# YichengDWu/tinyedm

Hardware: AMD Instinct MI355X
Metric: train imgs/sec CIFAR-10 32x32 bf16 (higher is better)
Workload: dtype bf16; 1 GPU; CIFAR-10 32x32 unconditional EDM2 U-Net (conf/cifar10.yaml, 35.6M params) full training step: diffuse+embed+denoiser fwd/bwd+loss+grad all-reduce+Adam+EMA; per_gpu_batch=128, global_batch=128, parallelism=dp1, conditional=False, step_launch=hipGraph replay, collective=none

## Files before the change

### tinyedm_amd/csrc/elementwise.hip

```cpp
#include "common.h"
#include <stdarg.h>
#include <stdio.h>

static thread_local char g_err[512] = "";
extern "C" void edm_set_error(const char* fmt, ...) {
  va_list ap;
  va_start(ap, fmt);
  vsnprintf(g_err, sizeof(g_err), fmt, ap);
  va_end(ap);
}
extern "C" const char* edm_last_error() { return g_err; }
extern "C" int edm_version() { return 1; }

static inline int cdiv(long a, long b) { return (int)((a + b - 1) / b); }
static inline int grid_for(long work, int block, int cap = 256 * 16) {
  long g = (work + block - 1) / block;
  if (g > cap) g = cap;
  if (g < 1) g = 1;
  return (int)g;
}

template <int LPP, bool POOL = false>
__global__ __launch_bounds__(256) void k_pnorm_silu_fwd(const bf16* __restrict__ x, bf16* __restrict__ xn,
                                                          bf16* __restrict__ a, float* __restrict__ dsave, int P,
                                                          int C, int Hp = 0, int Wp = 0) {
  constexpr int GPW = 64 / LPP;
  const int lane = threadIdx.x & 63, wave = threadIdx.x >> 6;
  const int lig = lane % LPP, grp = lane / LPP;
  const int CL = C >> 3;
  const float rsC = rsqrtf((float)C);
  const long stride = (long)gridDim.x * 4 * GPW;
  for (long p0 = ((long)blockIdx.x * 4 + wave) * GPW; p0 < P; p0 += stride) {
    const long p = p0 + grp;
    const bool pv = p < P;
    float v[2][8];
    float ss = 0.f;
#pragma unroll
    for (int it = 0; it < 2; ++it) {
      const int c8 = lig + it * LPP;
      if (pv && c8 < CL) {
        if constexpr (POOL) {
          const int w = (int)(p % Wp);
          const long t = p / Wp;
          const int h = (int)(t % Hp);
          const long b = t / Hp;
          const bf16* src = x + ((b * 2 * Hp + 2 * h) * 2 * Wp + 2 * w) * C + c8 * 8;
          const long row = (long)2 * Wp * C;
          float a1[8], a2[8], a3[8];
          load8(src, v[it]);
          load8(src + C, a1);
          load8(src + row, a2);
          load8(src + row + C, a3);
#pragma unroll
          for (int i = 0; i < 8; ++i) v[it][i] = (float)(bf16)(0.25f * (v[it][i] + a1[i] + a2[i] + a3[i]));
        } else {
          load8(x + p * C + c8 * 8, v[it]);
        }
#pragma unroll
        for (int i = 0; i < 8; ++i) ss += v[it][i] * v[it][i];
      }
    }
    ss = group_sum<LPP>(ss);
    const float d = NORM_EPS + sqrtf(ss) * rsC;
    const float inv = 1.0f / d;
#pragma unroll
    for (int it = 0; it < 2; ++it) {
      const int c8 = lig + it * LPP;
      if (pv && c8 < CL) {
        float o[8], s[8];
#pragma unroll
        for (int i = 0; i < 8; ++i) {
          o[i] = (float)(bf16)(v[it][i] * inv);
          s[i] = mp_silu_b(o[i]);
        }
        store8(xn + p * C + c8 * 8, o);
        store8(a + p * C + c8 * 8, s);
      }
    }
    if (pv && lig == 0) dsave[p] = d;
  }
}

template <int LPP, bool UP = false>
__global__ __launch_bounds__(256) void k_pnorm_silu_bwd(const bf16* __restrict__ xn, const float* __restrict__ dsave,
                                                          const bf16* __restrict__ gxn, float gs,
                                                          const bf16* __restrict__ ga, const bf16* __restrict__ gadd,
                                                          bf16* __restrict__ gx, int P, int C, int Hp = 0, int Wp = 0) {
  constexpr int GPW = 64 / LPP;
  const int lane = threadIdx.x & 63, wave = threadIdx.x >> 6;
  const int lig = lane % LPP, grp = lane / LPP;
  const int CL = C >> 3;
  const long stride = (long)gridDim.x * 4 * GPW;
  for (long p0 = ((long)blockIdx.x * 4 + wave) * GPW; p0 < P; p0 += stride) {
    const long p = p0 + grp;
    const bool pv = p < P;
    float y[2][8], g[2][8];
    float dot = 0.f;
#pragma unroll
    for (int it = 0; it < 2; ++it) {
      const int c8 = lig + it * LPP;
      if (pv && c8 < CL) {
        load8(xn + p * C + c8 * 8, y[it]);
        float t[8];
        if (gxn) {
          load8(gxn + p * C + c8 * 8, t);
#pragma unroll
          for (int i = 0; i < 8; ++i) g[it][i] = gs * t[i];
        } else {
#pragma unroll
          for (int i = 0; i < 8; ++i) g[it][i] = 0.f;
        }
        if (ga) {
          load8(ga + p * C + c8 * 8, t);
#pragma unroll
          for (int i = 0; i < 8; ++i) g[it][i] += mp_silu_grad_b(y[it][i]) * t[i];
        }
#pragma unroll
        for (int i = 0; i < 8; ++i) dot += g[it][i] * y[it][i];
      }
    }
    dot = group_sum<LPP>(dot);
    float d = pv ? dsave[p] : 1.f;
    float s = d - NORM_EPS;
    float coef = s > 0.f ? dot * d / ((float)C * s) : 0.f;
    float inv = 1.0f / d;
#pragma unroll
    for (int it = 0; it < 2; ++it) {
      const int c8 = lig + it * LPP;
      if (pv && c8 < CL) {
        float o[8];
#pragma unroll
        for (int i = 0; i < 8; ++i) o[i] = (g[it][i] - y[it][i] * coef) * inv;
        if constexpr (UP) {
          const int w = (int)(p % Wp);
          const long t2 = p / Wp;
          const int h = (int)(t2 % Hp);
          const long b = t2 / Hp;
          const long e0 = ((b * 2 * Hp + 2 * h) * 2 * Wp + 2 * w) * C + c8 * 8;
          const long row = (long)2 * Wp * C;
#pragma unroll
          for (int i = 0; i < 8; ++i) o[i] = 0.25f * (float)(bf16)o[i];
#pragma unroll
          for (int q = 0; q < 4; ++q) {
            const long e = e0 + (q >> 1) * row + (q & 1) * C;
            float r[8];
#pragma unroll
            for (int i = 0; i < 8; ++i) r[i] = o[i];
            if (gadd) {
              float t[8];
              load8(gadd + e, t);
#pragma unroll
              for (int i = 0; i < 8; ++i) r[i] += t[i];
            }
            store8(gx + e, r);
          }
          continue;
        }
        if (gadd) {
          float t[8];
          load8(gadd + p * C + c8 * 8, t);
#pragma unroll
          for (int i = 0; i < 8; ++i) o[i] += t[i];
        }
        store8(gx + p * C + c8 * 8, o);
      }
    }
  }
}

static int pick_lpp(int C) {
  int cl = C / 8;
  return cl <= 16 ? 16 : (cl <= 32 ? 32 : 64);
}

extern "C" int edm_pixelnorm_silu_fwd(const void* x, void* xn, void* a, float* dsave, long P, int C,
                                      hipStream_t st) {
  EDM_REQUIRE(P > 0 && P < (1L << 31) && C > 0 && C % 8 == 0 && C <= 1024, "pixelnorm_silu_fwd: bad P=%ld C=%d", P, C);
  int lpp = pick_lpp(C);
  int gpw = 64 / lpp;
  int grid = grid_for(P, 4 * gpw);
#define L(N) hipLaunchKernelGGL(k_pnorm_silu_fwd<N>, dim3(grid), dim3(256), 0, st, (const bf16*)x, (bf16*)xn, (bf16*)a, dsave, (int)P, C)
  if (lpp == 16) L(16); else if (lpp == 32) L(32); else L(64);
#undef L
  EDM_CHECK_LAUNCH("pixelnorm_silu_fwd");
  return EDM_OK;
}

extern "C" int edm_pool_pixelnorm_silu_fwd(const void* x, void* xn, void* a, float* dsave, int B, int Hp, int Wp, int C,
                                           hipStream_t st) {
  EDM_REQUIRE(x && xn && a && dsave && B > 0 && Hp > 0 && Wp > 0 && C > 0 && C % 8 == 0 && C <= 1024 &&
                  (long)B * Hp * Wp < (1L << 31), "pool_pixelnorm_silu_fwd: bad args");
  const long P = (long)B * Hp * Wp;
  int lpp = pick_lpp(C);
  int gpw = 64 / lpp;
  int grid = grid_for(P, 4 * gpw);
#define L(N) hipLaunchKernelGGL((k_pnorm_silu_fwd<N, true>), dim3(grid), dim3(256), 0, st, (const bf16*)x, (bf16*)xn, (bf16*)a, dsave, (int)P, C, Hp, Wp)
  if (lpp == 16) L(16); else if (lpp == 32) L(32); else L(64);
#undef L
  EDM_CHECK_LAUNCH("pool_pixelnorm_silu_fwd");
  return EDM_OK;
}
extern "C" int edm_pool_pixelnorm_silu_bwd(const void* xn, const float* dsave, const void* gxn, float gxn_scale,
                                           const void* ga, const void* gadd, void* gx, int B, int Hp, int Wp, int C,
                                           hipStream_t st) {
  EDM_REQUIRE(xn && dsave && gx && B > 0 && Hp > 0 && Wp > 0 && C > 0 && C % 8 == 0 && C <= 1024 &&
                  (long)B * Hp * Wp < (1L << 31), "pool_pixelnorm_silu_bwd: bad args");
  const long P = (long)B * Hp * Wp;
  int lpp = pick_lpp(C);
  int gpw = 64 / lpp;
  int grid = grid_for(P, 4 * gpw);
#define L(N) hipLaunchKernelGGL((k_pnorm_silu_bwd<N, true>), dim3(grid), dim3(256), 0, st, (const bf16*)xn, dsave, (const bf16*)gxn, gxn_scale, (const bf16*)ga, (const bf16*)gadd, (bf16*)gx, (int)P, C, Hp, Wp)
  if (lpp == 16) L(16); else if (lpp == 32) L(32); else L(64);
#undef L
  EDM_CHECK_LAUNCH("pool_pixelnorm_silu_bwd");
  return EDM_OK;
}

extern "C" int edm_pixelnorm_silu_bwd(const void* xn, const float* dsave, const void* gxn, float gxn_scale,
                                      const void* ga, const void* gadd, void* gx, long P, int C, hipStream_t st) {
  EDM_REQUIRE(P > 0 && P < (1L << 31) && C > 0 && C % 8 == 0 && C <= 1024, "pixelnorm_silu_bwd: bad P=%ld C=%d", P, C);
  int lpp = pick_lpp(C);
  int gpw = 64 / lpp;
  int grid = grid_for(P, 4 * gpw);
#define L(N) hipLaunchKernelGGL(k_pnorm_silu_bwd<N>, dim3(grid), dim3(256), 0, st, (const bf16*)xn, dsave, (const bf16*)gxn, gxn_scale, (const bf16*)ga, (const bf16*)gadd, (bf16*)gx, (int)P, C)
  if (lpp == 16) L(16); else if (lpp == 32) L(32); else L(64);
#undef L
  EDM_CHECK_LAUNCH("pixelnorm_silu_bwd");
  return EDM_OK;
}

__global__ void k_silu_fwd(const bf16* __restrict__ x, bf16* __restrict__ a, long n8) {
  for (long i = (long)blockIdx.x * blockDim.x + threadIdx.x; i < n8; i += (long)gridDim.x * blockDim.x) {
    float v[8];
    load8(x + i * 8, v);
#pragma unroll
    for (int j = 0; j < 8; ++j) v[j] = mp_silu_b(v[j]);
    store8(a + i * 8, v);
  }
}
__global__ void k_silu_bwd(const bf16* __restrict__ x, const bf16* __restrict__ ga, const bf16* __restrict__ ge,
                           float s, bf16* __restrict__ gx, long n8) {
  for (long i = (long)blockIdx.x * blockDim.x + threadIdx.x; i < n8; i += (long)gridDim.x * blockDim.x) {
    float v[8], g[8], e[8];
    load8(x + i * 8, v);
    load8(ga + i * 8, g);
    if (ge) load8(ge + i * 8, e);
#pragma unroll
    for (int j = 0; j < 8; ++j) g[j] = mp_silu_grad_b(v[j]) * g[j] + (ge ? s * e[j] : 0.f);
    store8(gx + i * 8, g);
  }
}
extern "C" int edm_silu_fwd(const void* x, void* a, long n, hipStream_t st) {
  EDM_REQUIRE(n > 0 && n % 8 == 0, "silu_fwd: n=%ld must be a positive multiple of 8", n);
  hipLaunchKernelGGL(k_silu_fwd, dim3(grid_for(n / 8, 256)), dim3(256), 0, st, (const bf16*)x, (bf16*)a, n / 8);
  EDM_CHECK_LAUNCH("silu_fwd");
  return EDM_OK;
}
extern "C" int edm_silu_bwd(const void* x, const void* ga, const void* gextra, float extra_scale, void* gx, long n,
                            hipStream_t st) {
  EDM_REQUIRE(n > 0 && n % 8 == 0, "silu_bwd: n=%ld must be a positive multiple of 8", n);
  hipLaunchKernelGGL(k_silu_bwd, dim3(grid_for(n / 8, 256)), dim3(256), 0, st, (const bf16*)x, (const bf16*)ga,
                     (const bf16*)gextra, extra_scale, (bf16*)gx, n / 8);
  EDM_CHECK_LAUNCH("silu_bwd");
  return EDM_OK;
}

__global__ void k_axpby(const bf16* __restrict__ a, float alpha, const bf16* __restrict__ b, float beta,
                        bf16* __restrict__ o, long n8) {
  for (long i = (long)blockIdx.x * blockDim.x + threadIdx.x; i < n8; i += (long)gridDim.x * blockDim.x) {
    float u[8], v[8];
    load8(a + i * 8, u);
    if (b) load8(b + i * 8, v);
#pragma unroll
    for (int j = 0; j < 8; ++j) u[j] = alpha * u[j] + (b ? beta * v[j] : 0.f);
    store8(o + i * 8, u);
  }
}
extern "C" int edm_axpby(const void* a, float alpha, const void* b, float beta, void* out, long n, hipStream_t st) {
  EDM_REQUIRE(n > 0 && n % 8 == 0, "axpby: n=%ld must be a positive multiple of 8", n);
  hipLaunchKernelGGL(k_axpby, dim3(grid_for(n / 8, 256)), dim3(256), 0, st, (const bf16*)a, alpha, (const bf16*)b,
                     beta, (bf16*)out, n / 8);
  EDM_CHECK_LAUNCH("axpby");
  return EDM_OK;
}


__global__ void k_mod_silu_drop_fwd(const bf16* __restrict__ r, const float* __restrict__ lin,
                                    const float* __restrict__ gain, bf16* __restrict__ a, int HW, int C, long n8,
                                    long lin_stride, float pdrop, uint32_t seed_lo, uint32_t seed_hi, uint32_t sub, uint32_t step,
                                    const StepParams* __restrict__ dyn) {
  if (dyn) { step = dyn->step; seed_lo = dyn->seed_lo; seed_hi = dyn->seed_hi; }
  const int CL = C >> 3;
  const float g = *gain;
  for (long i = (long)blockIdx.x * blockDim.x + threadIdx.x; i < n8; i += (long)gridDim.x * blockDim.x) {
    const int c8 = (int)(i % CL);
    const long pix = i / CL;
    const int b = (int)(pix / HW);
    float v[8];
    load8(r + i * 8, v);
    const float* lp = lin + (long)b * lin_stride + c8 * 8;
    const Keep8 keep = dropout_keep8(i, pdrop, sub, step, seed_lo, seed_hi);
    const float keep_scale = keep.scale;
#pragma unroll
    for (int j = 0; j < 8; ++j) {
      float m = lp[j] * g + 1.0f;
      float o = mp_silu_b(v[j] * m);
      if (pdrop > 0.f) o = keep[j] ? o * keep_scale : 0.f;
      v[j] = o;
    }
    store8(a + i * 8, v);
  }
}

__global__ void k_mod_silu_drop_bwd(const bf16* __restrict__ r, const float* __restrict__ lin,
                                    const float* __restrict__ gain, const bf16* __restrict__ ga,
                                    bf16* __restrict__ gr, float* __restrict__ gm, long gm_stride, int HW, int C, int PIXW,
                                    long lin_stride, float pdrop, uint32_t seed_lo, uint32_t seed_hi, uint32_t sub, uint32_t step,
                                    const StepParams* __restrict__ dyn) {
  extern __shared__ __attribute__((aligned(16))) float red[];
  if (dyn) { step = dyn->step; seed_lo = dyn->seed_lo; seed_hi = dyn->seed_hi; }
  const int CL = C >> 3;
  const int PS = blockDim.x / CL;
  const int c8 = threadIdx.x % CL, ps = threadIdx.x / CL;
  const int b = blockIdx.x;
  const int p_begin = blockIdx.y * PIXW;
  const int p_end = min(HW, p_begin + PIXW);
  const float g = *gain;
  float m[8], acc[8];
#pragma unroll
  for (int j = 0; j < 8; ++j) {
    m[j] = lin[(long)b * lin_stride + c8 * 8 + j] * g + 1.0f;
    acc[j] = 0.f;
  }
  for (int p = p_begin + ps; p < p_end; p += PS) {
    const long i = ((long)b * HW + p) * CL + c8;
    float v[8], gg[8];
    load8(r + i * 8, v);
    load8(ga + i * 8, gg);
    const Keep8 keep = dropout_keep8(i, pdrop, sub, step, seed_lo, seed_hi);
    const float keep_scale = keep.scale;
#pragma unroll
    for (int j = 0; j < 8; ++j) {
      const float u = (pdrop > 0.f && !keep[j]) ? 0.f : v[j];
      float gu = gg[j] * mp_silu_grad_b(u * m[j]);
      if (pdrop > 0.f) gu = keep[j] ? gu * keep_scale : 0.f;
      acc[j] += gu * u;
      gg[j] = gu * m[j];
    }
    store8(gr + i * 8, gg);
  }
#pragma unroll
  for (int j = 0; j < 8; ++j) red[ps * C + c8 * 8 + j] = acc[j];
  __syncthreads();
  for (int c = threadIdx.x; c < C; c += blockDim.x) {
    float s = 0.f;
    for (int q = 0; q < PS; ++q) s += red[q * C + c];
    atomicAdd(gm + (long)b * gm_stride + c, s);
  }
}
__global__ void k_mod_finish(const float* __restrict__ gm, const float* __restrict__ lin,
                             const float* __restrict__ gain, float* __restrict__ glin, float* __restrict__ ggain,
                             long n, int C, long lin_stride, long glin_stride) {
  const float g = *gain;
  float part = 0.f;
  for (long i = (long)blockIdx.x * blockDim.x + threadIdx.x; i < n; i += (long)gridDim.x * blockDim.x) {
    const long b = i / C;
    const int c = (int)(i - b * C);
    float v = gm[i];
    glin[b * glin_stride + c] = v * g;
    part += v * lin[b * lin_stride + c];
  }
  part = wave_sum(part);
  if ((threadIdx.x & 63) == 0) atomicAdd(ggain, part);
}

static int block_for_chunks(int CL) { return (256 / CL) * CL; }

extern "C" int edm_mod_silu_drop_fwd(const void* r, const float* lin, long lin_stride, const float* gain, void* a, int B,
                                     int HW, int C, float pdrop, unsigned long long seed, unsigned sub, unsigned step,
                                     const void* dyn, hipStream_t st) {
  EDM_REQUIRE(B > 0 && HW > 0 && C % 8 == 0 && C > 0 && pdrop >= 0.f && pdrop < 1.f && lin_stride >= C,
              "mod_silu_drop_fwd: bad args");
  long n8 = (long)B * HW * C / 8;
  hipLaunchKernelGGL(k_mod_silu_drop_fwd, dim3(grid_for(n8, 256)), dim3(256), 0, st, (const bf16*)r, lin, gain,
                     (bf16*)a, HW, C, n8, lin_stride, pdrop, (uint32_t)seed, (uint32_t)(seed >> 32), sub, step,
                     (const StepParams*)dyn);
  EDM_CHECK_LAUNCH("mod_silu_drop_fwd");
  return EDM_OK;
}

extern "C" int edm_mod_silu_drop_bwd(const void* r, const float* lin, long lin_stride, const float* gain,
                                     const void* ga, void* gr, float* gm, float* glin, long glin_stride, float* ggain,
                                     int B, int HW, int C, float pdrop, unsigned long long seed, unsigned sub,
                                     unsigned step, const void* dyn, hipStream_t st) {
  EDM_REQUIRE(B > 0 && HW > 0 && C % 8 == 0 && C > 0 && C <= 1024 && lin_stride >= C && glin_stride >= C,
              "mod_silu_drop_bwd: bad args");
  int CL = C / 8, block = block_for_chunks(CL), PS = block / CL;
  int PIXW = HW >= 256 ? 128 : HW;
  hipLaunchKernelGGL(k_mod_silu_drop_bwd, dim3(B, cdiv(HW, PIXW)), dim3(block), PS * C * sizeof(float), st,
                     (const bf16*)r, lin, gain, (const bf16*)ga, (bf16*)gr, gm, (long)C, HW, C, PIXW, lin_stride, pdrop,
                     (uint32_t)seed, (uint32_t)(seed >> 32), sub, step, (const StepParams*)dyn);
  EDM_CHECK_LAUNCH("mod_silu_drop_bwd");
  hipLaunchKernelGGL(k_mod_finish, dim3(grid_for((long)B * C, 256, 64)), dim3(256), 0, st, gm, lin, gain, glin,
                     ggain, (long)B * C, C, lin_stride, glin_stride);
  EDM_CHECK_LAUNCH("mod_finish");
  return EDM_OK;
}

extern "C" int edm_mod_silu_drop_bwd_raw(const void* r, const float* lin, long lin_stride, const float* gain,
                                         const void* ga, void* gr, float* gm, long gm_stride, int B, int HW, int C,
                                         float pdrop, unsigned long long seed, unsigned sub, unsigned step,
                                         const void* dyn, hipStream_t st) {
  EDM_REQUIRE(r && lin && gain && ga && gr && gm, "mod_silu_drop_bwd_raw: null pointer");
  EDM_REQUIRE(B > 0 && HW > 0 && C % 8 == 0 && C > 0 && C <= 1024 && lin_stride >= C && gm_stride >= C,
              "mod_silu_drop_bwd_raw: bad args");
  int CL = C / 8, block = block_for_chunks(CL), PS = block / CL;
  int PIXW = HW >= 256 ? 128 : HW;
  hipLaunchKernelGGL(k_mod_silu_drop_bwd, dim3(B, cdiv(HW, PIXW)), dim3(block), PS * C * sizeof(float), st,
                     (const bf16*)r, lin, gain, (const bf16*)ga, (bf16*)gr, gm, gm_stride, HW, C, PIXW, lin_stride, pdrop,
                     (uint32_t)seed, (uint32_t)(seed >> 32), sub, step, (const StepParams*)dyn);
  EDM_CHECK_LAUNCH("mod_silu_drop_bwd_raw");
  return EDM_OK;
}

extern "C" int edm_mod_finish(const float* gm, const float* lin, long lin_stride, const float* gain, float* glin,
                              long glin_stride, float* ggain, int B, int C, hipStream_t st) {
  EDM_REQUIRE(gm && lin && gain && glin && ggain && B > 0 && C > 0 && lin_stride >= C && glin_stride >= C,
              "mod_finish: bad args");
  hipLaunchKernelGGL(k_mod_finish, dim3(grid_for((long)B * C, 256, 64)), dim3(256), 0, st, gm, lin, gain, glin, ggain,
                     (long)B * C, C, lin_stride, glin_stride);
  EDM_CHECK_LAUNCH("mod_finish");
  return EDM_OK;
}

struct ModFinItem {
  const float* gain;
  float* ggain;
  int col0, C;
};
__global__ void k_mod_finish_multi(const float* __restrict__ gm, const float* __restrict__ lin, float* __restrict__ glin,
                                   long stride, const ModFinItem* __restrict__ items, int B) {
  const ModFinItem it = items[blockIdx.x];
  const float g = *it.gain;
  const long n = (long)B * it.C;
  float part = 0.f;
  for (long i = (long)blockIdx.y * blockDim.x + threadIdx.x; i < n; i += (long)gridDim.y * blockDim.x) {
    const long b = i / it.C;
    const long e = b * stride + it.col0 + (i - b * it.C);
    const float v = gm[e];
    glin[e] += v * g;
    part += v * lin[e];
  }
  __shared__ float red[4];
  part = wave_sum(part);
  if ((threadIdx.x & 63) == 0) red[threadIdx.x >> 6] = part;
  __syncthreads();
  if (threadIdx.x == 0) atomicAdd(it.ggain, red[0] + red[1] + red[2] + red[3]);
}
extern "C" int edm_mod_finish_multi(const float* gm_all, const float* lin_all, float* glin_all, long stride,
                                    const void* items_dev, int n_items, int B, hipStream_t st) {
  EDM_REQUIRE(gm_all && lin_all && glin_all && items_dev && n_items > 0 && n_items <= 4096 && B > 0 && stride > 0,
              "mod_finish_multi: bad args");
  hipLaunchKernelGGL(k_mod_finish_multi, dim3(n_items, 8), dim3(256), 0, st, gm_all, lin_all, glin_all, stride,
                     (const ModFinItem*)items_dev, B);
  EDM_CHECK_LAUNCH("mod_finish_multi");
  return EDM_OK;
}

__global__ void k_dropout_mask(uint8_t* __restrict__ mask, long n8, float pdrop, uint32_t seed_lo, uint32_t seed_hi,
                               uint32_t sub, uint32_t step) {
  for (long i = (long)blockIdx.x * blockDim.x + threadIdx.x; i < n8; i += (long)gridDim.x * blockDim.x) {
    const Keep8 keep = dropout_keep8(i, pdrop, sub, step, seed_lo, seed_hi);
#pragma unroll
    for (int j = 0; j < 8; ++j) mask[i * 8 + j] = keep[j] ? 1 : 0;
  }
}
extern "C" int edm_dropout_mask(unsigned char* mask, long n, float pdrop, unsigned long long seed, unsigned sub,
                                unsigned step, hipStream_t st) {
  EDM_REQUIRE(n > 0 && n % 8 == 0, "dropout_mask: n must be a multiple of 8");
  hipLaunchKernelGGL(k_dropout_mask, dim3(grid_for(n / 8, 256)), dim3(256), 0, st, mask, n / 8, pdrop,
                     (uint32_t)seed, (uint32_t)(seed >> 32), sub, step);
  EDM_CHECK_LAUNCH("dropout_mask");
  return EDM_OK;
}

__global__ void k_pool2(const bf16* __restrict__ x, bf16* __restrict__ y, int H, int W, int CL, long n8, float s) {
  for (long i = (long)blockIdx.x * blockDim.x + threadIdx.x; i < n8; i += (long)gridDim.x * blockDim.x) {
    int c8 = (int)(i % CL);
    long pix = i / CL;
    int w = (int)(pix % W);
    long t = pix / W;
    int h = (int)(t % H);
    long b = t / H;
    const long row = (long)2 * W * CL;
    const bf16* src = x + (((b * 2 * H + 2 * h) * 2 * W + 2 * w) * CL + c8) * 8;
    float a0[8], a1[8], a2[8], a3[8];
    load8(src, a0);
    load8(src + CL * 8, a1);
    load8(src + row * 8, a2);
    load8(src + row * 8 + CL * 8, a3);
#pragma unroll
    for (int j = 0; j < 8; ++j) a0[j] = s * (a0[j] + a1[j] + a2[j] + a3[j]);
    store8(y + i * 8, a0);
  }
}
__global__ void k_up2(const bf16* __restrict__ x, const bf16* __restrict__ add, bf16* __restrict__ y, int H, int W, int CL,
                      long n8, float s) {
  for (long i = (long)blockIdx.x * blockDim.x + threadIdx.x; i < n8; i += (long)gridDim.x * blockDim.x) {
    int c8 = (int)(i % CL);
    long pix = i / CL;
    int w = (int)(pix % W);
    long t = pix / W;
    int h = (int)(t % H);
    long b = t / H;
    const bf16* src = x + (((b * (H / 2) + h / 2) * (W / 2) + w / 2) * CL + c8) * 8;
    float a0[8];
    load8(src, a0);
    if (s != 1.0f) {
#pragma unroll
      for (int j = 0; j < 8; ++j) a0[j] *= s;
    }
    if (add) {
      float t[8];
      load8(add + i * 8, t);
#pragma unroll
      for (int j = 0; j < 8; ++j) a0[j] += t[j];
    }
    store8(y + i * 8, a0);
  }
}
__global__ void k_up2_silu(const bf16* __restrict__ x, bf16* __restrict__ y, bf16* __restrict__ a, int H, int W, int CL,
                           long n8) {
  for (long i = (long)blockIdx.x * blockDim.x + threadIdx.x; i < n8; i += (long)gridDim.x * blockDim.x) {
    int c8 = (int)(i % CL);
    long pix = i / CL;
    int w = (int)(pix % W);
    long t = pix / W;
    int h = (int)(t % H);
    long b = t / H;
    const u32x4 raw = *reinterpret_cast<const u32x4*>(x + (((b * (H / 2) + h / 2) * (W / 2) + w / 2) * CL + c8) * 8);
    *reinterpret_cast<u32x4*>(y + i * 8) = raw;
    const bf16x8 v = __builtin_bit_cast(bf16x8, raw);
    float f[8];
#pragma unroll
    for (int j = 0; j < 8; ++j) f[j] = mp_silu_b((float)v[j]);
    store8(a + i * 8, f);
  }
}
extern "C" int edm_up2_silu(const void* x, void* y, void* a, int B, int Hout, int Wout, int C, hipStream_t st) {
  EDM_REQUIRE(x && y && a && B > 0 && Hout > 0 && Wout > 0 && Hout % 2 == 0 && Wout % 2 == 0 && C % 8 == 0, "up2_silu: bad args");
  long n8 = (long)B * Hout * Wout * C / 8;
  hipLaunchKernelGGL(k_up2_silu, dim3(grid_for(n8, 256)), dim3(256), 0, st, (const bf16*)x, (bf16*)y, (bf16*)a, Hout, Wout,
                     C / 8, n8);
  EDM_CHECK_LAUNCH("up2_silu");
  return EDM_OK;
}
extern "C" int edm_pool2(const void* x, void* y, int B, int Hout, int Wout, int C, float scale, hipStream_t st) {
  EDM_REQUIRE(B > 0 && Hout > 0 && Wout > 0 && C % 8 == 0, "pool2: bad args");
  long n8 = (long)B * Hout * Wout * C / 8;
  hipLaunchKernelGGL(k_pool2, dim3(grid_for(n8, 256)), dim3(256), 0, st, (const bf16*)x, (bf16*)y, Hout, Wout, C / 8,
                     n8, scale);
  EDM_CHECK_LAUNCH("pool2");
  return EDM_OK;
}
extern "C" int edm_up2(const void* x, const void* add, void* y, int B, int Hout, int Wout, int C, float scale,
                       hipStream_t st) {
  EDM_REQUIRE(B > 0 && Hout > 0 && Wout > 0 && Hout % 2 == 0 && Wout % 2 == 0 && C % 8 == 0, "up2: bad args");
  long n8 = (long)B * Hout * Wout * C / 8;
  hipLaunchKernelGGL(k_up2, dim3(grid_for(n8, 256)), dim3(256), 0, st, (const bf16*)x, (const bf16*)add, (bf16*)y, Hout,
                     Wout, C / 8, n8, scale);
  EDM_CHECK_LAUNCH("up2");
  return EDM_OK;
}

__global__ __launch_bounds__(256) void k_reduce_hw_det(const bf16* __restrict__ x, long xs, const bf16* __restrict__ y,
                                                         long ys, float* __restrict__ out, int HW, int C, float scale) {
  __shared__ float red[32][65];
  const int b = blockIdx.x, c0 = blockIdx.y * 64;
  const int cl = threadIdx.x & 7, pl = threadIdx.x >> 3;
  const int c = c0 + cl * 8;
  const bool cok = c < C;
  float acc[8] = {0, 0, 0, 0, 0, 0, 0, 0};
  const long base = (long)b * HW;
  constexpr int UN = 16;
  for (int p0 = pl; p0 < HW; p0 += 32 * UN) {
    u32x4 v[UN], u[UN];
#pragma unroll
    for (int k = 0; k < UN; ++k) {
      const int p = p0 + 32 * k;
      const bool ok = cok && p < HW;
      v[k] = ok ? *reinterpret_cast<const u32x4*>(x + (base + p) * xs + c) : u32x4{0u, 0u, 0u, 0u};
      if (y) u[k] = ok ? *reinterpret_cast<const u32x4*>(y + (base + p) * ys + c) : u32x4{0u, 0u, 0u, 0u};
    }
#pragma unroll
    for (int k = 0; k < UN; ++k) {
      const bf16x8 a = __builtin_bit_cast(bf16x8, v[k]);
      if (y) {
        const bf16x8 b = __builtin_bit_cast(bf16x8, u[k]);
#pragma unroll
        for (int j = 0; j < 8; ++j) acc[j] += (float)a[j] * (float)b[j];
      } else {
#pragma unroll
        for (int j = 0; j < 8; ++j) acc[j] += (float)a[j];
      }
    }
  }
#pragma unroll
  for (int j = 0; j < 8; ++j) red[pl][cl * 8 + j] = acc[j];
  __syncthreads();
  if (threadIdx.x < 64 && c0 + (int)threadIdx.x < C) {
    float s = 0.f;
#pragma unroll
    for (int q = 0; q < 32; ++q) s += red[q][threadIdx.x];
    out[(long)b * C + c0 + threadIdx.x] = s * scale;
  }
}
extern "C" int edm_reduce_hw(const void* x, long x_stride, const void* y, long y_stride, float* out, int B, int HW,
                             int C, float scale, hipStream_t st) {
  EDM_REQUIRE(B > 0 && HW > 0 && C % 8 == 0 && C > 0 && C <= 4096 && x_stride % 8 == 0 && y_stride % 8 == 0,
              "reduce_hw: bad args");
  hipLaunchKernelGGL(k_reduce_hw_det, dim3(B, cdiv(C, 64)), dim3(256), 0, st, (const bf16*)x, x_stride, (const bf16*)y,
                     y_stride, out, HW, C, scale);
  EDM_CHECK_LAUNCH("reduce_hw");
  return EDM_OK;
}

__device__ __forceinline__ float strided_dot(const float* __restrict__ w, long stride, const float* v, int n) {
  float s = 0.f;
  int r = 0;
  for (; r + 16 <= n; r += 16) {
    float t[16];
#pragma unroll
    for (int k = 0; k < 16; ++k) t[k] = w[(long)(r + k) * stride];
#pragma unroll
    for (int k = 0; k < 16; ++k) s += t[k] * v[r + k];
  }
  for (; r < n; ++r) s += w[(long)r * stride] * v[r];
  return s;
}

__global__ void k_scalelong_fwd(const float* __restrict__ mean, const float* __restrict__ W1, const float* __restrict__ W2,
                                float* __restrict__ gate, float* __restrict__ z1save, int C, int R) {
  extern __shared__ __attribute__((aligned(16))) float sm[];
  float* m = sm;
  float* h = sm + C + 1;
  const int b = blockIdx.x;
  for (int c = threadIdx.x; c < C; c += blockDim.x) m[c] = mean[(long)b * C + c];
  if (threadIdx.x == 0) m[C] = 1.0f;
  __syncthreads();
  const int lane = threadIdx.x & 63, wave = threadIdx.x >> 6, nw = blockDim.x >> 6;
  for (int r = wave; r < R; r += nw) {
    float s = 0.f;
    for (int c = lane; c <= C; c += 64) s += W1[(long)r * (C + 1) + c] * m[c];
    s = wave_sum(s);
    if (lane == 0) {
      z1save[(long)b * R + r] = s;
      h[r] = mp_silu_f(s);
    }
  }
  __syncthreads();
  for (int c = threadIdx.x; c < C; c += blockDim.x) gate[(long)b * C + c] = sigmoidf_(strided_dot(W2 + (long)c * R, 1, h, R));
}
__global__ void k_scalelong_bwd(const float* __restrict__ mean, const float* __restrict__ W1, const float* __restrict__ W2,
                                const float* __restrict__ gate, const float* __restrict__ z1save,
                                const float* __restrict__ ggate, float* __restrict__ gmean, float* __restrict__ gW1,
                                float* __restrict__ gW2, int C, int R) {
  extern __shared__ __attribute__((aligned(16))) float sm[];
  float* m = sm;
  float* h = m + C + 1;
  float* gz2 = h + R;
  float* gz1 = gz2 + C;
  const int b = blockIdx.x;
  for (int c = threadIdx.x; c < C; c += blockDim.x) {
    m[c] = mean[(long)b * C + c];
    float g = gate[(long)b * C + c];
    gz2[c] = ggate[(long)b * C + c] * g * (1.0f - g);
  }
  if (threadIdx.x == 0) m[C] = 1.0f;
  for (int r = threadIdx.x; r < R; r += blockDim.x) h[r] = mp_silu_f(z1save[(long)b * R + r]);
  __syncthreads();
  for (int i = threadIdx.x; i < C * R; i += blockDim.x) atomicAdd(gW2 + i, gz2[i / R] * h[i % R]);
  const int lane = threadIdx.x & 63, wave = threadIdx.x >> 6, nw = blockDim.x >> 6;
  for (int r = wave; r < R; r += nw) {
    float s = 0.f;
    for (int c = lane; c < C; c += 64) s += W2[(long)c * R + r] * gz2[c];
    s = wave_sum(s);
    if (lane == 0) gz1[r] = s * mp_silu_grad_f(z1save[(long)b * R + r]);
  }
  __syncthreads();
  for (int i = threadIdx.x; i < R * (C + 1); i += blockDim.x) atomicAdd(gW1 + i, gz1[i / (C + 1)] * m[i % (C + 1)]);
  for (int c = threadIdx.x; c < C; c += blockDim.x) {
    float s = 0.f;
    for (int r = 0; r < R; ++r) s += W1[(long)r * (C + 1) + c] * gz1[r];
    gmean[(long)b * C + c] = s;
  }
}
extern "C" int edm_scalelong_fwd(const float* mean, const float* W1h, const float* W2h, float* gate, float* z1save,
                                 int B, int C, int R, hipStream_t st) {
  EDM_REQUIRE(B > 0 && C > 0 && R > 0 && C <= 4096, "scalelong_fwd: bad args");
  hipLaunchKernelGGL(k_scalelong_fwd, dim3(B), dim3(256), (C + 1 + R) * sizeof(float), st, mean, W1h, W2h, gate,
                     z1save, C, R);
  EDM_CHECK_LAUNCH("scalelong_fwd");
  return EDM_OK;
}
extern "C" int edm_scalelong_bwd(const float* mean, const float* W1h, const float* W2h, const float* gate,
                                 const float* z1save, const float* ggate, float* gmean, float* gW1h, float* gW2h,
                                 int B, int C, int R, hipStream_t st) {
  EDM_REQUIRE(B > 0 && C > 0 && R > 0 && C <= 4096, "scalelong_bwd: bad args");
  hipLaunchKernelGGL(k_scalelong_bwd, dim3(B), dim3(256), (2 * C + 1 + 2 * R) * sizeof(float), st, mean, W1h, W2h,
                     gate, z1save, ggate, gmean, gW1h, gW2h, C, R);
  EDM_CHECK_LAUNCH("scalelong_bwd");
  return EDM_OK;
}

template <bool MUL>
__device__ __forceinline__ void sample_reduce(const bf16* __restrict__ x, long xs, const bf16* __restrict__ y, long ys,
                                              int HW, int C, float* red, float* out_lds, float scale) {
  const int lpr = C >> 3;
  const int rpp = blockDim.x / lpr;
  const int cl = threadIdx.x % lpr, rg = threadIdx.x / lpr;
  float acc[8] = {0, 0, 0, 0, 0, 0, 0, 0};
  if (rg < rpp) {
    constexpr int UN = 8;
    for (int p0 = rg; p0 < HW; p0 += rpp * UN) {
      u32x4 v[UN], u[UN];
#pragma unroll
      for (int k = 0; k < UN; ++k) {
        const int p = p0 + rpp * k;
        const bool ok = p < HW;
        v[k] = ok ? *reinterpret_cast<const u32x4*>(x + (long)p * xs + cl * 8) : u32x4{0u, 0u, 0u, 0u};
        if (MUL) u[k] = ok ? *reinterpret_cast<const u32x4*>(y + (long)p * ys + cl * 8) : u32x4{0u, 0u, 0u, 0u};
      }
#pragma unroll
      for (int k = 0; k < UN; ++k) {
        const bf16x8 a = __builtin_bit_cast(bf16x8, v[k]);
        if (MUL) {
          const bf16x8 b = __builtin_bit_cast(bf16x8, u[k]);
#pragma unroll
          for (int j = 0; j < 8; ++j) acc[j] += (float)a[j] * (float)b[j];
        } else {
#pragma unroll
          for (int j = 0; j < 8; ++j) acc[j] += (float)a[j];
        }
      }
    }
#pragma unroll
    for (int j = 0; j < 8; ++j) red[rg * C + cl * 8 + j] = acc[j];
  }
  __syncthreads();
  for (int c = threadIdx.x; c < C; c += blockDim.x) {
    float s = 0.f;
    for (int q = 0; q < rpp; ++q) s += red[q * C + c];
    out_lds[c] = s * scale;
  }
  __syncthreads();
}

template <bool KEEP = false>
__device__ __forceinline__ void skip_gate_fwd_body(const bf16* __restrict__ skip, const float* __restrict__ W1,
                                                   const float* __restrict__ W2, float* __restrict__ mean,
                                                   float* __restrict__ gate, float* __restrict__ z1save, int HW,
                                                   int C, int R, int b) {
  extern __shared__ __attribute__((aligned(16))) float sm[];
  const int rpp = blockDim.x / (C >> 3);
  float* red = sm;
  float* m = sm + rpp * C;
  float* h = m + C + 1;
  sample_reduce<false>(skip + (long)b * HW * C, C, nullptr, 0, HW, C, red, m, 1.0f / (float)HW);
  for (int c = threadIdx.x; c < C; c += blockDim.x) mean[(long)b * C + c] = m[c];
  if (threadIdx.x == 0) m[C] = 1.0f;
  __syncthreads();
  const int lane = threadIdx.x & 63, wave = threadIdx.x >> 6, nw = blockDim.x >> 6;
  for (int r = wave < nw ? wave : R; r < R; r += nw) {
    float s = 0.f;
    for (int c = lane; c <= C; c += 64) s += W1[(long)r * (C + 1) + c] * m[c];
    s = wave_sum(s);
    if (lane == 0) {
      z1save[(long)b * R + r] = s;
      h[r] = mp_silu_f(s);
    }
  }
  __syncthreads();
  for (int c = threadIdx.x; c < C; c += blockDim.x) {
    const float gv = sigmoidf_(strided_dot(W2 + (long)c * R, 1, h, R));
    gate[(long)b * C + c] = gv;
    if (KEEP) red[c] = gv;
  }
}
__global__ __launch_bounds__(1024) void k_skip_gate_fwd(const bf16* __restrict__ skip, const float* __restrict__ W1,
                                                          const float* __restrict__ W2, float* __restrict__ mean,
                                                          float* __restrict__ gate, float* __restrict__ z1save, int HW,
                                                          int C, int R) {
  skip_gate_fwd_body(skip, W1, W2, mean, gate, z1save, HW, C, R, blockIdx.x);
}
constexpr int MAXSGF = 32;
struct SgfItem {
  const bf16* skip;
  const float* W1;
  const float* W2;
  float* mean;
  float* gate;
  float* z1;
  bf16* cat;
  bf16* sil;
  int Ci, pad;
  int B, HW, R, blk0;
};
struct SgfGroup {
  SgfItem it[MAXSGF];
  int n, C, pad[2];
};
__global__ __launch_bounds__(1024) void k_skip_gate_fwd_multi(const SgfGroup* __restrict__ g) {
  int k = 0;
  const int n = g->n;
  while (k + 1 < n && (int)blockIdx.x >= g->it[k + 1].blk0) ++k;
  const SgfItem it = g->it[k];
  const int C = g->C, b = (int)blockIdx.x - it.blk0;
  skip_gate_fwd_body<true>(it.skip, it.W1, it.W2, it.mean, it.gate, it.z1, it.HW, C, it.R, b);
  if (it.cat == nullptr) return;
  __syncthreads();
  extern __shared__ __attribute__((aligned(16))) float sm[];
  const int CLs = C >> 3;
  const long ld = it.Ci + C;
  const bf16* __restrict__ sk = it.skip + (long)b * it.HW * C;
  bf16* __restrict__ cat = it.cat + (long)b * it.HW * ld + it.Ci;
  bf16* __restrict__ sil = it.sil ? it.sil + (long)b * it.HW * ld + it.Ci : nullptr;
  const int n8 = it.HW * CLs;
  for (int i = threadIdx.x; i < n8; i += blockDim.x) {
    const int cs = (i % CLs) * 8;
    const int pix = i / CLs;
    float v[8];
    load8(sk + (long)pix * C + cs, v);
#pragma unroll
    for (int j = 0; j < 8; ++j) v[j] = (float)(bf16)(v[j] * sm[cs + j]);
    store8(cat + (long)pix * ld + cs, v);
    if (sil) {
#pragma unroll
      for (int j = 0; j < 8; ++j) v[j] = mp_silu_b(v[j]);
      store8(sil + (long)pix * ld + cs, v);
    }
  }
}
__device__ __forceinline__ void skip_gate_bwd_body(const bf16* __restrict__ gcat, long gs, const bf16* __restrict__ skip,
                                                   const float* __restrict__ W1, const float* __restrict__ W2,
                                                   const float* __restrict__ gate, const float* __restrict__ z1save,
                                                   float* __restrict__ gmean, float* __restrict__ ws, int HW, int C,
                                                   int R, int b) {
  extern __shared__ __attribute__((aligned(16))) float sm[];
  const int rpp = blockDim.x / (C >> 3);
  float* red = sm;
  float* gz2 = sm + rpp * C;
  float* gz1 = gz2 + C;
  float* wsb = ws + (long)b * (C + 2 * R);
  sample_reduce<true>(gcat + (long)b * HW * gs, gs, skip + (long)b * HW * C, C, HW, C, red, gz2, 1.0f);
  for (int c = threadIdx.x; c < C; c += blockDim.x) {
    const float g = gate[(long)b * C + c];
    gz2[c] *= g * (1.0f - g);
    wsb[c] = gz2[c];
  }
  for (int r = threadIdx.x; r < R; r += blockDim.x) wsb[C + R + r] = mp_silu_f(z1save[(long)b * R + r]);
  __syncthreads();
  const int lane = threadIdx.x & 63, wave = threadIdx.x >> 6, nw = blockDim.x >> 6;
  for (int r = wave < nw ? wave : R; r < R; r += nw) {
    float s = 0.f;
    for (int c = lane; c < C; c += 64) s += W2[(long)c * R + r] * gz2[c];
    s = wave_sum(s);
    if (lane == 0) {
      gz1[r] = s * mp_silu_grad_f(z1save[(long)b * R + r]);
      wsb[C + r] = gz1[r];
    }
  }
  __syncthreads();
  for (int c = threadIdx.x; c < C; c += blockDim.x) gmean[(long)b * C + c] = strided_dot(W1 + c, C + 1, gz1, R);
}
__global__ __launch_bounds__(1024) void k_skip_gate_bwd(const bf16* __restrict__ gcat, long gs, const bf16* __restrict__ skip,
                                                          const float* __restrict__ W1, const float* __restrict__ W2,
                                                          const float* __restrict__ gate, const float* __restrict__ z1save,
                                                          float* __restrict__ gmean, float* __restrict__ ws, int HW, int C,
                                                          int R) {
  skip_gate_bwd_body(gcat, gs, skip, W1, W2, gate, z1save, gmean, ws, HW, C, R, blockIdx.x);
}
struct SgbItem {
  const bf16* gcat;
  long gs;
  const bf16* skip;
  const float* W1;
  const float* W2;
  const float* gate;
  const float* z1;
  float* gmean;
  float* ws;
  bf16* gskip;
  int B, HW, R, blk0;
};
struct SgbGroup {
  SgbItem it[MAXSGF];
  int n, C, pad[2];
};
__global__ __launch_bounds__(1024) void k_skip_gate_bwd_multi(const SgbGroup* __restrict__ g) {
  int k = 0;
  const int n = g->n;
  while (k + 1 < n && (int)blockIdx.x >= g->it[k + 1].blk0) ++k;
  const SgbItem it = g->it[k];
  const int C = g->C, b = (int)blockIdx.x - it.blk0;
  skip_gate_bwd_body(it.gcat, it.gs, it.skip, it.W1, it.W2, it.gate, it.z1, it.gmean, it.ws, it.HW, C, it.R, b);
  if (it.gskip == nullptr) return;
  __syncthreads();
  const int CLs = C >> 3;
  const float inv_hw = 1.0f / (float)it.HW;
  const bf16* __restrict__ gc = it.gcat + (long)b * it.HW * it.gs;
  bf16* __restrict__ out = it.gskip + (long)b * it.HW * C;
  const float* gp0 = it.gate + (long)b * C;
  const float* mp0 = it.gmean + (long)b * C;
  const int n8 = it.HW * CLs;
  for (int i = threadIdx.x; i < n8; i += blockDim.x) {
    const int cs = (i % CLs) * 8;
    const int pix = i / CLs;
    float v[8];
    load8(gc + (long)pix * it.gs + cs, v);
    const float* gp = gp0 + cs;
    const float* mp = mp0 + cs;
#pragma unroll
    for (int j = 0; j < 8; ++j) v[j] = v[j] * gp[j] + mp[j] * inv_hw;
    store8(out + (long)pix * C + cs, v);
  }
}
__device__ __forceinline__ void skip_gate_wgrad_body(const float* __restrict__ ws, const float* __restrict__ mean,
                                                     float* __restrict__ gW1, float* __restrict__ gW2, int B, int C, int R,
                                                     int CT, int BC, int blk) {
  extern __shared__ __attribute__((aligned(16))) float sm[];
  float* A = sm;
  float* Bm = sm + 4 * BC;
  const int W = C + 2 * R;
  const bool second = blk >= CT;
  const int c0 = (second ? blk - CT : blk) * 4;
  const int ncol = second ? C + 1 : C;
  const int boff = second ? C : C + R;
  constexpr int MAXO = 16;
  float acc[MAXO];
#pragma unroll
  for (int k = 0; k < MAXO; ++k) acc[k] = 0.f;
  for (int b0 = 0; b0 < B; b0 += BC) {
    const int nb = min(BC, B - b0);
    if (b0) __syncthreads();
    for (int i = threadIdx.x; i < 4 * nb; i += blockDim.x) {
      const int b = b0 + (i >> 2), c = c0 + (i & 3);
      float v = 0.f;
      if (c < ncol) v = second ? (c < C ? mean[(long)b * C + c] : 1.0f) : ws[(long)b * W + c];
      A[i] = v;
    }
    for (int i = threadIdx.x; i < nb * R; i += blockDim.x) Bm[i] = ws[(long)(b0 + i / R) * W + boff + i % R];
    __syncthreads();
#pragma unroll
    for (int k = 0; k < MAXO; ++k) {
      const int o = threadIdx.x + k * 256;
      if (o < 4 * R) {
        const int cc = o / R, r = o % R;
        float s = acc[k];
        for (int b = 0; b < nb; ++b) s += A[b * 4 + cc] * Bm[b * R + r];
        acc[k] = s;
      }
    }
  }
#pragma unroll
  for (int k = 0; k < MAXO; ++k) {
    const int o = threadIdx.x + k * 256;
    if (o >= 4 * R) continue;
    const int cc = o / R, r = o % R;
    if (c0 + cc >= ncol) continue;
    if (second) gW1[(long)r * (C + 1) + c0 + cc] = acc[k];
    else gW2[(long)(c0 + cc) * R + r] = acc[k];
  }
}
__global__ __launch_bounds__(256) void k_skip_gate_wgrad(const float* __restrict__ ws, const float* __restrict__ mean,
                                                           float* __restrict__ gW1, float* __restrict__ gW2, int B, int C,
                                                           int R, int CT, int BC) {
  skip_gate_wgrad_body(ws, mean, gW1, gW2, B, C, R, CT, BC, blockIdx.x);
}
constexpr int MAXSG = 32;
struct SgItem {
  const float* ws;
  const float* mean;
  float* gW1;
  float* gW2;
  int B, C, R, blk0;
};
struct SgGroup {
  SgItem it[MAXSG];
  int n, pad[3];
};
__global__ __launch_bounds__(256) void k_skip_gate_wgrad_multi(const SgGroup* __restrict__ g) {
  int k = 0;
  const int n = g->n;
  while (k + 1 < n && (int)blockIdx.x >= g->it[k + 1].blk0) ++k;
  const SgItem it = g->it[k];
  const int CT = (it.C + 3) / 4;
  const int BC = it.B < 16384 / (it.R + 4) ? it.B : 16384 / (it.R + 4);
  skip_gate_wgrad_body(it.ws, it.mean, it.gW1, it.gW2, it.B, it.C, it.R, CT, BC, (int)blockIdx.x - it.blk0);
}
static inline int skip_gate_threads(int C) {
  const int lpr = C / 8;
  int t = 1024 / lpr * lpr;
  return t < 64 ? 0 : t;
}
extern "C" int edm_skip_gate_fwd(const void* skip, const float* W1h, const float* W2h, float* mean, float* gate,
                                 float* z1save, int B, int HW, int C, int R, hipStream_t st) {
  EDM_REQUIRE(skip && W1h && W2h && mean && gate && z1save, "skip_gate_fwd: null pointer");
  EDM_REQUIRE(B > 0 && HW > 0 && C > 0 && C % 8 == 0 && C <= 4096 && R > 0 && R <= 1024, "skip_gate_fwd: bad args");
  const int threads = skip_gate_threads(C);
  EDM_REQUIRE(threads > 0, "skip_gate_fwd: C too large");
  const size_t lds = ((size_t)(threads / (C / 8)) * C + C + 1 + R) * sizeof(float);
  hipLaunchKernelGGL(k_skip_gate_fwd, dim3(B), dim3(threads), lds, st, (const bf16*)skip, W1h, W2h, mean, gate, z1save,
                     HW, C, R);
  EDM_CHECK_LAUNCH("skip_gate_fwd");
  return EDM_OK;
}
struct edm_skip_gate_fwd_item_ {
  const void* skip;
  const float* W1h;
  const float* W2h;
  float* mean;
  float* gate;
  float* z1save;
  void* cat;
  void* silu_out;
  int B, HW, C, R, Ci, pad;
};
extern "C" long edm_skip_gate_fwd_multi_table_bytes(void) { return (long)sizeof(SgfGroup); }
extern "C" int edm_skip_gate_fwd_multi(const void* items_, int n, void* table_host, void* table_dev, int defer_upload,
                                       hipStream_t st) {
  const edm_skip_gate_fwd_item_* items = (const edm_skip_gate_fwd_item_*)items_;
  EDM_REQUIRE(items && n > 0 && n <= MAXSGF, "skip_gate_fwd_multi: need 1..%d gates, got %d", MAXSGF, n);
  SgfGroup g;
  g.n = n;
  g.C = items[0].C;
  g.pad[0] = g.pad[1] = 0;
  const int C = g.C;
  EDM_REQUIRE(C > 0 && C % 8 == 0 && C <= 4096, "skip_gate_fwd_multi: bad channel count %d", C);
  const int threads = skip_gate_threads(C);
  EDM_REQUIRE(threads > 0, "skip_gate_fwd_multi: C too large");
  long blk = 0;
  int rmax = 0;
  for (int k = 0; k < n; ++k) {
    const edm_skip_gate_fwd_item_& a = items[k];
    EDM_REQUIRE(a.skip && a.W1h && a.W2h && a.mean && a.gate && a.z1save, "skip_gate_fwd_multi: null pointer (gate %d)", k);
    EDM_REQUIRE(a.C == C, "skip_gate_fwd_multi: the gates of one launch share a channel count (%d vs %d)", a.C, C);
    EDM_REQUIRE(a.B > 0 && a.HW > 0 && a.R > 0 && a.R <= 1024, "skip_gate_fwd_multi: bad item %d", k);
    EDM_REQUIRE(a.cat ? (a.Ci > 0 && a.Ci % 8 == 0) : (a.silu_out == nullptr),
                "skip_gate_fwd_multi: cat needs Ci %% 8 == 0 (gate %d); silu_out needs cat", k);
    g.it[k] = SgfItem{(const bf16*)a.skip, a.W1h, a.W2h, a.mean, a.gate, a.z1save, (bf16*)a.cat, (bf16*)a.silu_out, a.Ci, 0,
                      a.B, a.HW, a.R, (int)blk};
    blk += a.B;
    EDM_REQUIRE(blk < (1L << 30), "skip_gate_fwd_multi: grid too large");
    if (a.R > rmax) rmax = a.R;
  }
  for (int k = n; k < MAXSGF; ++k)
    g.it[k] = SgfItem{nullptr, nullptr, nullptr, nullptr, nullptr, nullptr, nullptr, nullptr, 0, 0, 0, 0, 0, (int)blk};
  const size_t lds = ((size_t)(threads / (C / 8)) * C + C + 1 + rmax) * sizeof(float);
  EDM_UPLOAD_TABLE(table_dev, table_host, &g, sizeof(SgfGroup), st, "skip_gate_fwd_multi", defer_upload);
  hipLaunchKernelGGL(k_skip_gate_fwd_multi, dim3((unsigned)blk), dim3(threads), lds, st, (const SgfGroup*)table_dev);
  EDM_CHECK_LAUNCH("skip_gate_fwd_multi");
  return EDM_OK;
}
extern "C" int edm_skip_gate_bwd(const void* gcat, long gcat_stride, int c_off, const void* skip, const float* mean,
                                 const float* W1h, const float* W2h, const float* gate, const float* z1save, float* gmean,
                                 float* gW1h, float* gW2h, float* ws, int B, int HW, int C, int R, hipStream_t st) {
  EDM_REQUIRE(gcat && skip && mean && W1h && W2h && gate && z1save && gmean && ws && (!gW1h == !gW2h), "skip_gate_bwd: null pointer");
  EDM_REQUIRE(B > 0 && HW > 0 && C > 0 && C % 8 == 0 && C <= 4096 && R > 0 && R <= 1024 && c_off >= 0 && c_off % 8 == 0 &&
                  gcat_stride >= c_off + C && gcat_stride % 8 == 0, "skip_gate_bwd: bad args");
  const int threads = skip_gate_threads(C);
  EDM_REQUIRE(threads > 0, "skip_gate_bwd: C too large");
  const size_t lds = ((size_t)(threads / (C / 8)) * C + C + R) * sizeof(float);
  hipLaunchKernelGGL(k_skip_gate_bwd, dim3(B), dim3(threads), lds, st, (const bf16*)gcat + c_off, gcat_stride,
                     (const bf16*)skip, W1h, W2h, gate, z1save, gmean, ws, HW, C, R);
  if (gW1h) {
    const int CT = (C + 3) / 4, CT1 = (C + 4) / 4;
    const int BC = B < 16384 / (R + 4) ? B : 16384 / (R + 4);
    const size_t lds2 = ((size_t)4 * BC + (size_t)BC * R) * sizeof(float);
    hipLaunchKernelGGL(k_skip_gate_wgrad, dim3(CT + CT1), dim3(256), lds2, st, ws, mean, gW1h, gW2h, B, C, R, CT, BC);
  }
  EDM_CHECK_LAUNCH("skip_gate_bwd");
  return EDM_OK;
}

struct edm_skip_gate_bwd_item_ {
  const void* gcat;
  long gcat_stride;
  const void* skip;
  const float* W1h;
  const float* W2h;
  const float* gate;
  const float* z1save;
  float* gmean;
  float* ws;
  void* gskip;
  int c_off, B, HW, C, R, pad;
};
extern "C" int edm_skip_gate_bwd_multi(const void* items_, int n, void* table_host, void* table_dev, int defer_upload,
                                       hipStream_t st) {
  const edm_skip_gate_bwd_item_* items = (const edm_skip_gate_bwd_item_*)items_;
  EDM_REQUIRE(items && n > 0 && n <= MAXSGF, "skip_gate_bwd_multi: need 1..%d gates, got %d", MAXSGF, n);
  SgbGroup g;
  g.n = n;
  g.C = items[0].C;
  g.pad[0] = g.pad[1] = 0;
  const int C = g.C;
  EDM_REQUIRE(C > 0 && C % 8 == 0 && C <= 4096, "skip_gate_bwd_multi: bad channel count %d", C);
  const int threads = skip_gate_threads(C);
  EDM_REQUIRE(threads > 0, "skip_gate_bwd_multi: C too large");
  long blk = 0;
  int rmax = 0;
  for (int k = 0; k < n; ++k) {
    const edm_skip_gate_bwd_item_& a = items[k];
    EDM_REQUIRE(a.gcat && a.skip && a.W1h && a.W2h && a.gate && a.z1save && a.gmean && a.ws,
                "skip_gate_bwd_multi: null pointer (gate %d)", k);
    EDM_REQUIRE(a.C == C, "skip_gate_bwd_multi: the gates of one launch share a channel count (%d vs %d)", a.C, C);
    EDM_REQUIRE(a.B > 0 && a.HW > 0 && a.R > 0 && a.R <= 1024 && a.c_off >= 0 && a.c_off % 8 == 0 &&
                    a.gcat_stride >= a.c_off + C && a.gcat_stride % 8 == 0, "skip_gate_bwd_multi: bad item %d", k);
    g.it[k] = SgbItem{(const bf16*)a.gcat + a.c_off, a.gcat_stride, (const bf16*)a.skip, a.W1h, a.W2h, a.gate, a.z1save,
                      a.gmean, a.ws, (bf16*)a.gskip, a.B, a.HW, a.R, (int)blk};
    blk += a.B;
    EDM_REQUIRE(blk < (1L << 30), "skip_gate_bwd_multi: grid too large");
    if (a.R > rmax) rmax = a.R;
  }
  for (int k = n; k < MAXSGF; ++k)
    g.it[k] = SgbItem{nullptr, 0, nullptr, nullptr, nullptr, nullptr, nullptr, nullptr, nullptr, nullptr, 0, 0, 0, (int)blk};
  const size_t lds = ((size_t)(threads / (C / 8)) * C + C + rmax) * sizeof(float);
  EDM_UPLOAD_TABLE(table_dev, table_host, &g, sizeof(SgbGroup), st, "skip_gate_bwd_multi", defer_upload);
  hipLaunchKernelGGL(k_skip_gate_bwd_multi, dim3((unsigned)blk), dim3(threads), lds, st, (const SgbGroup*)table_dev);
  EDM_CHECK_LAUNCH("skip_gate_bwd_multi");
  return EDM_OK;
}
struct edm_skip_gate_wgrad_item_ {
  const float* ws;
  const float* mean;
  float* gW1h;
  float* gW2h;
  int B, C, R, pad;
};
extern "C" long edm_skip_gate_wgrad_multi_table_bytes(void) { return (long)sizeof(SgGroup); }
extern "C" int edm_skip_gate_wgrad_multi(const void* items_, int n, void* table_host, void* table_dev, int defer_upload,
                                         hipStream_t st) {
  const edm_skip_gate_wgrad_item_* items = (const edm_skip_gate_wgrad_item_*)items_;
  EDM_REQUIRE(items && n > 0 && n <= MAXSG, "skip_gate_wgrad_multi: need 1..%d gates, got %d", MAXSG, n);
  SgGroup g;
  g.n = n;
  int blk = 0;
  size_t lds = 0;
  for (int k = 0; k < n; ++k) {
    const edm_skip_gate_wgrad_item_& a = items[k];
    EDM_REQUIRE(a.ws && a.mean && a.gW1h && a.gW2h && a.B > 0 && a.C > 0 && a.C % 8 == 0 && a.C <= 4096 && a.R > 0 && a.R <= 1024,
                "skip_gate_wgrad_multi: bad item %d", k);
    g.it[k] = SgItem{a.ws, a.mean, a.gW1h, a.gW2h, a.B, a.C, a.R, blk};
    blk += (a.C + 3) / 4 + (a.C + 4) / 4;
    const int BC = a.B < 16384 / (a.R + 4) ? a.B : 16384 / (a.R + 4);
    const size_t need = ((size_t)4 * BC + (size_t)BC * a.R) * sizeof(float);
    if (need > lds) lds = need;
  }
  EDM_MAX_LDS(k_skip_gate_wgrad_multi, 128 * 1024);
  EDM_UPLOAD_TABLE(table_dev, table_host, &g, sizeof(SgGroup), st, "skip_gate_wgrad_multi", defer_upload);
  hipLaunchKernelGGL(k_skip_gate_wgrad_multi, dim3(blk), dim3(256), lds, st, (const SgGroup*)table_dev);
  EDM_CHECK_LAUNCH("skip_gate_wgrad_multi");
  return EDM_OK;
}

__global__ void k_concat_gate_fwd(const bf16* __restrict__ inp, const bf16* __restrict__ skip,
                                  const float* __restrict__ gate, bf16* __restrict__ cat, bf16* __restrict__ sil,
                                  int HW, int Ci, int Cs, long n8) {
  const int CLt = (Ci + Cs) >> 3, CLi = Ci >> 3;
  for (long i = (long)blockIdx.x * blockDim.x + threadIdx.x; i < n8; i += (long)gridDim.x * blockDim.x) {
    int c8 = (int)(i % CLt);
    long pix = i / CLt;
    float v[8];
    if (c8 < CLi) {
      load8(inp + pix * Ci + c8 * 8, v);
    } else {
      int cs = (c8 - CLi) * 8;
      int b = (int)(pix / HW);
      load8(skip + pix * Cs + cs, v);
      const float* gp = gate + (long)b * Cs + cs;
#pragma unroll
      for (int j = 0; j < 8; ++j) v[j] = (float)(bf16)(v[j] * gp[j]);
    }
    store8(cat + i * 8, v);
    if (sil) {
#pragma unroll
      for (int j = 0; j < 8; ++j) v[j] = mp_silu_b(v[j]);
      store8(sil + i * 8, v);
    }
  }
}
__global__ void k_concat_gate_bwd(const bf16* __restrict__ gcat, const float* __restrict__ gate,
                                  const float* __restrict__ gmean, bf16* __restrict__ ginp, bf16* __restrict__ gskip,
                                  int HW, int Ci, int Cs, long n8, float inv_hw) {
  const int CLt = (Ci + Cs) >> 3, CLi = Ci >> 3;
  for (long i = (long)blockIdx.x * blockDim.x + threadIdx.x; i < n8; i += (long)gridDim.x * blockDim.x) {
    int c8 = (int)(i % CLt);
    long pix = i / CLt;
    float v[8];
    load8(gcat + i * 8, v);
    if (c8 < CLi) {
      store8(ginp + pix * Ci + c8 * 8, v);
    } else {
      int cs = (c8 - CLi) * 8;
      int b = (int)(pix / HW);
      const float* gp = gate + (long)b * Cs + cs;
      const float* mp = gmean + (long)b * Cs + cs;
#pragma unroll
      for (int j = 0; j < 8; ++j) v[j] = v[j] * gp[j] + mp[j] * inv_hw;
      store8(gskip + pix * Cs + cs, v);
    }
  }
}
__global__ void k_skip_half_fwd(const bf16* __restrict__ skip, const float* __restrict__ gate, bf16* __restrict__ cat,
                                bf16* __restrict__ sil, int HW, int Ci, int Cs, long n8) {
  const int CLs = Cs >> 3;
  const long ld = Ci + Cs;
  for (long i = (long)blockIdx.x * blockDim.x + threadIdx.x; i < n8; i += (long)gridDim.x * blockDim.x) {
    const int cs = (int)(i % CLs) * 8;
    const long pix = i / CLs;
    const int b = (int)(pix / HW);
    float v[8];
    load8(skip + pix * Cs + cs, v);
    const float* gp = gate + (long)b * Cs + cs;
#pragma unroll
    for (int j = 0; j < 8; ++j) v[j] = (float)(bf16)(v[j] * gp[j]);
    store8(cat + pix * ld + Ci + cs, v);
    if (sil) {
#pragma unroll
      for (int j = 0; j < 8; ++j) v[j] = mp_silu_b(v[j]);
      store8(sil + pix * ld + Ci + cs, v);
    }
  }
}
__device__ __forceinline__ void skip_half_bwd_body(const bf16* __restrict__ gcs, const float* __restrict__ gate,
                                                   const float* __restrict__ gmean, bf16* __restrict__ gskip, int HW, int Cs,
                                                   long n8, float inv_hw, long first, long stride) {
  const int CLs = Cs >> 3;
  for (long i = first; i < n8; i += stride) {
    const int cs = (int)(i % CLs) * 8;
    const int b = (int)((i / CLs) / HW);
    float v[8];
    load8(gcs + i * 8, v);
    const float* gp = gate + (long)b * Cs + cs;
    const float* mp = gmean + (long)b * Cs + cs;
#pragma unroll
    for (int j = 0; j < 8; ++j) v[j] = v[j] * gp[j] + mp[j] * inv_hw;
    store8(gskip + i * 8, v);
  }
}
__global__ void k_skip_half_bwd(const bf16* __restrict__ gcs, const float* __restrict__ gate,
                                const float* __restrict__ gmean, bf16* __restrict__ gskip, int HW, int Cs, long n8,
                                float inv_hw) {
  skip_half_bwd_body(gcs, gate, gmean, gskip, HW, Cs, n8, inv_hw, (long)blockIdx.x * blockDim.x + threadIdx.x,
                     (long)gridDim.x * blockDim.x);
}
struct ShbItem {
  const bf16* gcs;
  const float* gate;
  const float* gmean;
  bf16* gskip;
  long n8;
  float inv_hw;
  int HW, Cs, blk0, nblk, pad;
};
struct ShbGroup {
  ShbItem it[MAXSGF];
  int n, pad[3];
};
__global__ void k_skip_half_bwd_multi(const ShbGroup* __restrict__ g) {
  int k = 0;
  const int n = g->n;
  while (k + 1 < n && (int)blockIdx.x >= g->it[k + 1].blk0) ++k;
  const ShbItem it = g->it[k];
  skip_half_bwd_body(it.gcs, it.gate, it.gmean, it.gskip, it.HW, it.Cs, it.n8, it.inv_hw,
                     (long)((int)blockIdx.x - it.blk0) * blockDim.x + threadIdx.x, (long)it.nblk * blockDim.x);
}
extern "C" int edm_skip_half_fwd(const void* skip, const float* gate, void* cat, void* silu_out, int B, int HW, int Ci,
                                 int Cs, hipStream_t st) {
  EDM_REQUIRE(skip && gate && cat, "skip_half_fwd: null pointer");
  EDM_REQUIRE(B > 0 && HW > 0 && Ci % 8 == 0 && Cs % 8 == 0 && Ci > 0 && Cs > 0, "skip_half_fwd: bad args");
  long n8 = (long)B * HW * Cs / 8;
  hipLaunchKernelGGL(k_skip_half_fwd, dim3(grid_for(n8, 256)), dim3(256), 0, st, (const bf16*)skip, gate, (bf16*)cat,
                     (bf16*)silu_out, HW, Ci, Cs, n8);
  EDM_CHECK_LAUNCH("skip_half_fwd");
  return EDM_OK;
}
extern "C" int edm_skip_half_bwd(const void* gcs, const float* gate, const float* gmean, void* gskip, int B, int HW, int Cs,
                                 hipStream_t st) {
  EDM_REQUIRE(gcs && gate && gmean && gskip, "skip_half_bwd: null pointer");
  EDM_REQUIRE(B > 0 && HW > 0 && Cs % 8 == 0 && Cs > 0, "skip_half_bwd: bad args");
  long n8 = (long)B * HW * Cs / 8;
  hipLaunchKernelGGL(k_skip_half_bwd, dim3(grid_for(n8, 256)), dim3(256), 0, st, (const bf16*)gcs, gate, gmean,
                     (bf16*)gskip, HW, Cs, n8, 1.0f / (float)HW);
  EDM_CHECK_LAUNCH("skip_half_bwd");
  return EDM_OK;
}
extern "C" long edm_skip_gate_bwd_multi_table_bytes(void) {
  return (long)(sizeof(SgbGroup) > sizeof(ShbGroup) ? sizeof(SgbGroup) : sizeof(ShbGroup));
}
struct edm_skip_half_bwd_item_ {
  const void* gcs;
  const float* gate;
  const float* gmean;
  void* gskip;
  int B, HW, Cs, pad;
};
extern "C" int edm_skip_half_bwd_multi(const void* items_, int n, void* table_host, void* table_dev, int defer_upload,
                                       hipStream_t st) {
  const edm_skip_half_bwd_item_* items = (const edm_skip_half_bwd_item_*)items_;
  EDM_REQUIRE(items && n > 0 && n <= MAXSGF, "skip_half_bwd_multi: need 1..%d tensors, got %d", MAXSGF, n);
  ShbGroup g;
  g.n = n;
  g.pad[0] = g.pad[1] = g.pad[2] = 0;
  long blk = 0;
  for (int k = 0; k < n; ++k) {
    const edm_skip_half_bwd_item_& a = items[k];
    EDM_REQUIRE(a.gcs && a.gate && a.gmean && a.gskip, "skip_half_bwd_multi: null pointer (tensor %d)", k);
    EDM_REQUIRE(a.B > 0 && a.HW > 0 && a.Cs % 8 == 0 && a.Cs > 0, "skip_half_bwd_multi: bad item %d", k);
    const long n8 = (long)a.B * a.HW * a.Cs / 8;
    const int nblk = grid_for(n8, 256);
    g.it[k] = ShbItem{(const bf16*)a.gcs, a.gate, a.gmean, (bf16*)a.gskip, n8, 1.0f / (float)a.HW, a.HW, a.Cs, (int)blk, nblk, 0};
    blk += nblk;
    EDM_REQUIRE(blk < (1L << 30), "skip_half_bwd_multi: grid too large");
  }
  for (int k = n; k < MAXSGF; ++k) g.it[k] = ShbItem{nullptr, nullptr, nullptr, nullptr, 0, 0.f, 1, 8, (int)blk, 0, 0};
  EDM_UPLOAD_TABLE(table_dev, table_host, &g, sizeof(ShbGroup), st, "skip_half_bwd_multi", defer_upload);
  hipLaunchKernelGGL(k_skip_half_bwd_multi, dim3((unsigned)blk), dim3(256), 0, st, (const ShbGroup*)table_dev);
  EDM_CHECK_LAUNCH("skip_half_bwd_multi");
  return EDM_OK;
}

extern "C" int edm_concat_gate_fwd(const void* inp, const void* skip, const float* gate, void* cat, void* silu_out,
                                   int B, int HW, int Ci, int Cs, hipStream_t st) {
  EDM_REQUIRE(B > 0 && HW > 0 && Ci % 8 == 0 && Cs % 8 == 0 && Ci > 0 && Cs > 0, "concat_gate_fwd: bad args");
  long n8 = (long)B * HW * (Ci + Cs) / 8;
  hipLaunchKernelGGL(k_concat_gate_fwd, dim3(grid_for(n8, 256)), dim3(256), 0, st, (const bf16*)inp,
                     (const bf16*)skip, gate, (bf16*)cat, (bf16*)silu_out, HW, Ci, Cs, n8);
  EDM_CHECK_LAUNCH("concat_gate_fwd");
  return EDM_OK;
}
extern "C" int edm_concat_gate_bwd(const void* gcat, const float* gate, const float* gmean, void* ginp, void* gskip,
                                   int B, int HW, int Ci, int Cs, hipStream_t st) {
  EDM_REQUIRE(B > 0 && HW > 0 && Ci % 8 == 0 && Cs % 8 == 0 && Ci > 0 && Cs > 0, "concat_gate_bwd: bad args");
  long n8 = (long)B * HW * (Ci + Cs) / 8;
  hipLaunchKernelGGL(k_concat_gate_bwd, dim3(grid_for(n8, 256)), dim3(256), 0, st, (const bf16*)gcat, gate, gmean,
                     (bf16*)ginp, (bf16*)gskip, HW, Ci, Cs, n8, 1.0f / (float)HW);
  EDM_CHECK_LAUNCH("concat_gate_bwd");
  return EDM_OK;
}

__global__ void k_precond_in(const float* __restrict__ noisy, const float* __restrict__ sigma, int sstride, float sd,
                             bf16* __restrict__ out, int Cimg, int HW, int CP, long npix) {
  for (long p = (long)blockIdx.x * blockDim.x + threadIdx.x; p < npix; p += (long)gridDim.x * blockDim.x) {
    long b = p / HW;
    int hw = (int)(p % HW);
    float s = sigma[b * sstride];
    float cin = rsqrtf(sd * sd + s * s);
    bf16* o = out + p * CP;
    for (int c0 = 0; c0 < CP; c0 += 8) {
      float v[8];
#pragma unroll
      for (int j = 0; j < 8; ++j) {
        int c = c0 + j;
        v[j] = c < Cimg ? cin * noisy[(b * Cimg + c) * HW + hw] : (c == Cimg ? 1.0f : 0.0f);
      }
      store8(o + c0, v);
    }
  }
}
extern "C" int edm_precond_in(const float* noisy, const float* sigma, int sigma_stride, float sigma_data, void* out,
                              int B, int Cimg, int HW, int CP, hipStream_t st) {
  EDM_REQUIRE(B > 0 && Cimg > 0 && HW > 0 && CP % 8 == 0 && CP > Cimg && (sigma_stride == 0 || sigma_stride == 1),
              "precond_in: bad args");
  long npix = (long)B * HW;
  hipLaunchKernelGGL(k_precond_in, dim3(grid_for(npix, 256)), dim3(256), 0, st, noisy, sigma, sigma_stride,
                     sigma_data, (bf16*)out, Cimg, HW, CP, npix);
  EDM_CHECK_LAUNCH("precond_in");
  return EDM_OK;
}

template <int LPP>
__global__ __launch_bounds__(256) void k_conv_out_fwd(const bf16* __restrict__ x, const float* __restrict__ wh,
                                                        const float* __restrict__ gain_out,
                                                        const float* __restrict__ noisy,
                                                        const float* __restrict__ sigma, int sstride, float sd,
                                                        float* __restrict__ D, float* __restrict__ Fraw, int HW,
                                                        int C, int Co, long npix) {
  constexpr int GPW = 64 / LPP;
  const int lane = threadIdx.x & 63, wave = threadIdx.x >> 6;
  const int lig = lane % LPP, grp = lane / LPP;
  const int CL = C >> 3;
  const float go = *gain_out;
  const long stride = (long)gridDim.x * 4 * GPW;
  for (long p0 = ((long)blockIdx.x * 4 + wave) * GPW; p0 < npix; p0 += stride) {
    const long p = p0 + grp;
    const bool pv = p < npix;
    float acc[8] = {0, 0, 0, 0, 0, 0, 0, 0};
    if (pv) {
      for (int c8 = lig; c8 < CL; c8 += LPP) {
        float v[8];
        load8(x + p * C + c8 * 8, v);
#pragma unroll
        for (int o = 0; o < 8; ++o) {
          if (o < Co) {
            const float* wp = wh + (long)o * C + c8 * 8;
#pragma unroll
            for (int j = 0; j < 8; ++j) acc[o] += v[j] * wp[j];
          }
        }
      }
    }
#pragma unroll
    for (int o = 0; o < 8; ++o)
      if (o < Co) acc[o] = group_sum<LPP>(acc[o]);
    if (pv && lig == 0) {
      const int b = (int)p / HW, hw = (int)p - b * HW;
      float s = sigma[b * sstride];
      float den = s * s + sd * sd;
      float cskip = sd * sd / den, cout = s * sd * rsqrtf(den);
#pragma unroll
      for (int o = 0; o < 8; ++o) {
        if (o < Co) {
          long idx = ((long)b * Co + o) * HW + hw;
          if (Fraw) Fraw[idx] = acc[o];
          D[idx] = acc[o] * go * cout + noisy[idx] * cskip;
        }
      }
    }
  }
}
extern "C" int edm_conv_out_fwd(const void* x, const float* w_hat, const float* gain_out, const float* noisy,
                                const float* sigma, int sigma_stride, float sigma_data, float* D, float* Fraw, int B,
                                int HW, int C, int Co, hipStream_t st) {
  EDM_REQUIRE(B > 0 && HW > 0 && C % 8 == 0 && Co >= 1 && Co <= 8 && (sigma_stride == 0 || sigma_stride == 1),
              "conv_out_fwd: bad args (Co<=8 required)");
  long npix = (long)B * HW;
  EDM_REQUIRE(npix < (1L << 31), "conv_out_fwd: too many pixels");
  hipLaunchKernelGGL(k_conv_out_fwd<8>, dim3(grid_for(npix, 32)), dim3(256), 0, st, (const bf16*)x, w_hat, gain_out,
                     noisy, sigma, sigma_stride, sigma_data, D, Fraw, HW, C, Co, npix);
  EDM_CHECK_LAUNCH("conv_out_fwd");
  return EDM_OK;
}

__global__ void k_conv_out_bwd_x(const float* __restrict__ dD, const float* __restrict__ wh,
                                 const float* __restrict__ gain_out, const float* __restrict__ sigma, int sstride,
                                 float sd, bf16* __restrict__ gx, int HW, int C, int Co, long n8) {
  const unsigned CL = (unsigned)C >> 3, uHW = (unsigned)HW;
  const float go = *gain_out;
  for (unsigned i = blockIdx.x * blockDim.x + threadIdx.x; i < (unsigned)n8; i += gridDim.x * blockDim.x) {
    const unsigned p = i / CL, c8 = i - p * CL;
    const unsigned b = p / uHW, hw = p - b * uHW;
    float s = sigma[b * sstride];
    float cout = s * sd * rsqrtf(s * s + sd * sd) * go;
    float v[8] = {0, 0, 0, 0, 0, 0, 0, 0};
    for (int o = 0; o < Co; ++o) {
      float df = dD[((long)b * Co + o) * HW + hw] * cout;
      const float* wp = wh + (long)o * C + c8 * 8;
#pragma unroll
      for (int j = 0; j < 8; ++j) v[j] += df * wp[j];
    }
    store8(gx + (long)i * 8, v);
  }
}
__global__ void k_conv_out_bwd_w(const bf16* __restrict__ x, const float* __restrict__ dD,
                                 const float* __restrict__ Fraw, const float* __restrict__ gain_out,
                                 const float* __restrict__ sigma, int sstride, float sd, float* __restrict__ gwh,
                                 float* __restrict__ ggain, int HW, int C, int Co, long npix, int PIXW) {
  extern __shared__ __attribute__((aligned(16))) float red[];
  const int CL = C >> 3;
  const int PS = blockDim.x / CL;
  const int c8 = threadIdx.x % CL, ps = threadIdx.x / CL;
  const long p0 = (long)blockIdx.x * PIXW, p1 = min(npix, p0 + PIXW);
  const float go = *gain_out;
  float acc[8][8];
#pragma unroll
  for (int o = 0; o < 8; ++o)
#pragma unroll
    for (int j = 0; j < 8; ++j) acc[o][j] = 0.f;
  float gg = 0.f;
  int p = (int)p0 + ps;
  const int pend = (int)p1;
  int b = p / HW, hw = p - b * HW;
  float cout = 0.f;
  {
    const float s = sigma[(p < pend ? b : 0) * sstride];
    cout = s * sd * rsqrtf(s * s + sd * sd);
  }
  float vn[8] = {0, 0, 0, 0, 0, 0, 0, 0}, dn[8] = {0, 0, 0, 0, 0, 0, 0, 0}, fn[8] = {0, 0, 0, 0, 0, 0, 0, 0};
  auto fetch = [&](int pp, int bb, int hh) {
    load8(x + (long)pp * C + c8 * 8, vn);
#pragma unroll
    for (int o = 0; o < 8; ++o)
      if (o < Co) {
        const long idx = ((long)bb * Co + o) * HW + hh;
        dn[o] = dD[idx];
        if (c8 == 0) fn[o] = Fraw[idx];
      }
  };
  if (p < pend) fetch(p, b, hw);
  while (p < pend) {
    float v[8], dd[8], ff[8];
#pragma unroll
    for (int j = 0; j < 8; ++j) { v[j] = vn[j]; dd[j] = dn[j]; ff[j] = fn[j]; }
    const float cur = cout;
    p += PS;
    hw += PS;
    if (hw >= HW) {
      do {
        hw -= HW;
        ++b;
      } while (hw >= HW);
      if (p < pend) {
        const float s = sigma[b * sstride];
        cout = s * sd * rsqrtf(s * s + sd * sd);
      }
    }
    if (p < pend) fetch(p, b, hw);
#pragma unroll
    for (int o = 0; o < 8; ++o) {
      if (o < Co) {
        float d = dd[o] * cur;
        if (c8 == 0) gg += d * ff[o];
        d *= go;
#pragma unroll
        for (int j = 0; j < 8; ++j) acc[o][j] += d * v[j];
      }
    }
  }
#pragma unroll
  for (int o = 0; o < 8; ++o)
    if (o < Co) {
#pragma unroll
      for (int j = 0; j < 8; ++j) red[(ps * Co + o) * C + c8 * 8 + j] = acc[o][j];
    }
  __syncthreads();
  for (int e = threadIdx.x; e < Co * C; e += blockDim.x) {
    float sacc = 0.f;
    for (int q = 0; q < PS; ++q) sacc += red[q * Co * C + e];
    atomicAdd(gwh + e, sacc);
  }
  if (c8 == 0) atomicAdd(ggain, gg);
}
extern "C" int edm_conv_out_bwd(const void* x, const float* w_hat, const float* gain_out, const float* Fraw,
                                const float* dD, const float* sigma, int sigma_stride, float sigma_data, void* gx,
                                float* gw_hat, float* ggain, int B, int HW, int C, int Co, hipStream_t st) {
  EDM_REQUIRE(B > 0 && HW > 0 && C % 8 == 0 && Co >= 1 && Co <= 8 && (sigma_stride == 0 || sigma_stride == 1),
              "conv_out_bwd: bad args");
  long npix = (long)B * HW, n8 = npix * C / 8;
  EDM_REQUIRE(n8 < (1L << 31), "conv_out_bwd: too many elements (32-bit index arithmetic)");
  hipLaunchKernelGGL(k_conv_out_bwd_x, dim3(grid_for(n8, 256)), dim3(256), 0, st, dD, w_hat, gain_out, sigma,
                     sigma_stride, sigma_data, (bf16*)gx, HW, C, Co, n8);
  EDM_CHECK_LAUNCH("conv_out_bwd_x");
  if (gw_hat) {
    const int CL = C / 8;
    EDM_REQUIRE(CL <= 256, "conv_out_bwd: C=%d too large", C);
    int block = (256 / CL) * CL, PS = block / CL;
    while (PS > 1 && (size_t)PS * Co * C * sizeof(float) > 48 * 1024) { --PS; block = PS * CL; }
    const int PIXW = 256;
    hipLaunchKernelGGL(k_conv_out_bwd_w, dim3(cdiv(npix, PIXW)), dim3(block), (size_t)PS * Co * C * sizeof(float), st,
                       (const bf16*)x, dD, Fraw, gain_out, sigma, sigma_stride, sigma_data, gw_hat, ggain, HW, C, Co,
                       npix, PIXW);
    EDM_CHECK_LAUNCH("conv_out_bwd_w");
  }
  return EDM_OK;
}

__global__ void k_nchw_f32_to_nhwc_bf16(const float* __restrict__ x, bf16* __restrict__ y, int C, int HW, long n8) {
  const int CL = C >> 3;
  for (long i = (long)blockIdx.x * blockDim.x + threadIdx.x; i < n8; i += (long)gridDim.x * blockDim.x) {
    int c8 = (int)(i % CL);
    long p = i / CL;
    long b = p / HW;
    int hw = (int)(p % HW);
    float v[8];
#pragma unroll
    for (int j = 0; j < 8; ++j) v[j] = x[(b * C + c8 * 8 + j) * HW + hw];
    store8(y + i * 8, v);
  }
}
__global__ void k_nhwc_bf16_to_nchw_f32(const bf16* __restrict__ x, float* __restrict__ y, int C, int HW, long n8) {
  const int CL = C >> 3;
  for (long i = (long)blockIdx.x * blockDim.x + threadIdx.x; i < n8; i += (long)gridDim.x * blockDim.x) {
    int c8 = (int)(i % CL);
    long p = i / CL;
    long b = p / HW;
    int hw = (int)(p % HW);
    float v[8];
    load8(x + i * 8, v);
#pragma unroll
    for (int j = 0; j < 8; ++j) y[(b * C + c8 * 8 + j) * HW + hw] = v[j];
  }
}
extern "C" int edm_nchw_to_nhwc_bf16(const float* x, void* y, int B, int C, int HW, hipStream_t st) {
  EDM_REQUIRE(B > 0 && C % 8 == 0 && HW > 0, "nchw_to_nhwc_bf16: bad args");
  long n8 = (long)B * HW * C / 8;
  hipLaunchKernelGGL(k_nchw_f32_to_nhwc_bf16, dim3(grid_for(n8, 256)), dim3(256), 0, st, x, (bf16*)y, C, HW, n8);
  EDM_CHECK_LAUNCH("nchw_to_nhwc_bf16");
  return EDM_OK;
}
extern "C" int edm_nhwc_bf16_to_nchw(const void* x, float* y, int B, int C, int HW, hipStream_t st) {
  EDM_REQUIRE(B > 0 && C % 8 == 0 && HW > 0, "nhwc_bf16_to_nchw: bad args");
  long n8 = (long)B * HW * C / 8;
  hipLaunchKernelGGL(k_nhwc_bf16_to_nchw_f32, dim3(grid_for(n8, 256)), dim3(256), 0, st, (const bf16*)x, y, C, HW, n8);
  EDM_CHECK_LAUNCH("nhwc_bf16_to_nchw");
  return EDM_OK;
}
```

### tinyedm_amd/csrc/tail_lowrank.hip

```cpp
#include "common.h"

typedef __attribute__((ext_vector_type(2))) float f32x2;

constexpr size_t LOWRANK_LDS_MAX = 60 * 1024;
static size_t dgrad_lds(int Co, int C, int W, int R, bool fused) {
  const int CL = C / 8, PS = ((256 / CL) * CL) / CL, TP = (W + 3) / 4 * 4 + 4;
  return ((size_t)Co * 9 * C + (size_t)Co * (R + 2) * TP + (fused ? (size_t)PS * C : 0)) * sizeof(float);
}
static size_t wgrad_lds(int Co, int taps, int C, int W, int R) {
  const int halo = taps == 9 ? 1 : 0;
  return ((size_t)Co * taps * C + (size_t)Co * (R + 2 * halo) * (W + 2 * halo)) * sizeof(float);
}
extern "C" int edm_lowrank_supported(int C, int Co, int W, int taps) {
  if (C <= 0 || C % 8 || C > 1024 || Co < 1 || Co > 8 || W <= 0 || (taps != 1 && taps != 9)) return 0;
  if (wgrad_lds(Co, taps, C, W, 1) > LOWRANK_LDS_MAX) return 0;
  return taps == 1 || dgrad_lds(Co, C, W, 1, true) <= LOWRANK_LDS_MAX;
}

__global__ void k_lowrank_df(const float* __restrict__ dD, const float* __restrict__ Fraw,
                             const float* __restrict__ gain_out, const float* __restrict__ sigma, int sstride, float sd,
                             float* __restrict__ dF, float* __restrict__ aux, int CoHW, long n) {
  const float go = *gain_out;
  for (long i = (long)blockIdx.x * blockDim.x + threadIdx.x; i < n; i += (long)gridDim.x * blockDim.x) {
    const int b = (int)(i / CoHW);
    const float s = sigma[b * sstride];
    const float c = s * sd * rsqrtf(s * s + sd * sd);
    const float d = dD[i];
    dF[i] = d * (c * go);
    if (aux) aux[i] = (d * c) * Fraw[i];
  }
}

extern "C" int edm_lowrank_df(const float* dD, const float* Fraw, const float* gain_out, const float* sigma,
                              int sigma_stride, float sigma_data, float* dF, float* aux, int B, int Co, int HW,
                              hipStream_t st) {
  EDM_REQUIRE(dD && gain_out && sigma && dF && (!aux || Fraw), "lowrank_df: null pointer");
  EDM_REQUIRE(B > 0 && HW > 0 && Co >= 1 && Co <= 8 && (sigma_stride == 0 || sigma_stride == 1), "lowrank_df: bad args");
  EDM_REQUIRE((long)Co * HW < (1L << 31), "lowrank_df: sample too large");
  const long n = (long)B * Co * HW;
  const long blocks = (n + 255) / 256;
  hipLaunchKernelGGL(k_lowrank_df, dim3((unsigned)(blocks < 2048 ? blocks : 2048)), dim3(256), 0, st, dD, Fraw, gain_out,
                     sigma, sigma_stride, sigma_data, dF, aux, Co * HW, n);
  EDM_CHECK_LAUNCH("lowrank_df");
  return EDM_OK;
}

template <int CO, bool FUSED>
__global__ __launch_bounds__(256, 4) void k_lowrank_dgrad3x3(const float* __restrict__ dF, const float* __restrict__ Wc,
                                                          float scale, bf16* __restrict__ ga, const bf16* __restrict__ U,
                                                          const float* __restrict__ lin, long lin_stride,
                                                          const float* __restrict__ gain, bf16* __restrict__ gr,
                                                          float* __restrict__ gm, long gm_stride, float pdrop,
                                                          uint32_t seed_lo, uint32_t seed_hi, uint32_t sub, uint32_t step,
                                                          int u_marks, const StepParams* __restrict__ dyn, int H, int W,
                                                          int C, int R, int TP) {
  extern __shared__ __attribute__((aligned(16))) float sm[];
  float* wl = sm;
  float* tl = wl + CO * 9 * C;
  float* red = tl + CO * (R + 2) * TP;
  const int CL = C >> 3;
  const int PS = blockDim.x / CL;
  const int c8 = threadIdx.x % CL, ps = threadIdx.x / CL;
  const int b = blockIdx.y, y0 = blockIdx.x * R;
  const int rows = min(R, H - y0);
  for (int i = threadIdx.x; i < CO * 9 * C / 4; i += blockDim.x)
    reinterpret_cast<f32x4*>(wl)[i] = reinterpret_cast<const f32x4*>(Wc)[i];
  for (int i = threadIdx.x; i < CO * (R + 2) * TP; i += blockDim.x) {
    const int o = i / ((R + 2) * TP), rem = i - o * (R + 2) * TP;
    const int ry = rem / TP, cx = rem - ry * TP;
    const int y = y0 + ry - 1, x = cx - 1;
    float v = 0.f;
    if (y >= 0 && y < H && x >= 0 && x < W) v = dF[(((long)b * CO + o) * H + y) * W + x];
    tl[i] = v;
  }
  __syncthreads();
  ModEpilogue m{};
  float mv[8], part[8];
  if constexpr (FUSED) {
    m.pdrop = pdrop; m.seed_lo = seed_lo; m.seed_hi = seed_hi; m.sub = sub; m.step = step; m.u_marks = u_marks; m.dyn = dyn;
    apply_dyn(m);
    const float g = *gain;
#pragma unroll
    for (int j = 0; j < 8; ++j) {
      mv[j] = lin[(long)b * lin_stride + c8 * 8 + j] * g + 1.0f;
      part[j] = 0.f;
    }
  }
  const int NSX = (W + 3) >> 2;
  const int nstrips = rows * NSX;
  for (int s = ps; s < nstrips; s += PS) {
    const int ry = s / NSX, x0 = (s - ry * NSX) * 4;
    const long p = ((long)b * H + y0 + ry) * W + x0;
    u32x4 ub[4];
    if constexpr (FUSED) {
#pragma unroll
      for (int k = 0; k < 4; ++k) {
        ub[k] = u32x4{0u, 0u, 0u, 0u};
        if (x0 + k < W) ub[k] = *reinterpret_cast<const u32x4*>(U + (p + k) * C + c8 * 8);
      }
    }
    f32x2 acc[4][4];
#pragma unroll
    for (int k = 0; k < 4; ++k)
#pragma unroll
      for (int j = 0; j < 4; ++j) acc[k][j] = f32x2{0.f, 0.f};
#pragma unroll 1
    for (int g = 0; g < 3 * CO; ++g) {
      const int ky = g / CO, o = g - ky * CO;
      {
        const float* tp = tl + (o * (R + 2) + ry + 2 - ky) * TP + x0;
        float dd[6];
#pragma unroll
        for (int j = 0; j < 6; ++j) dd[j] = tp[j];
#pragma unroll
        for (int kx = 0; kx < 3; ++kx) {
          const float* wp = wl + (o * 9 + ky * 3 + kx) * C + c8 * 8;
          const f32x4 w0 = *reinterpret_cast<const f32x4*>(wp), w1 = *reinterpret_cast<const f32x4*>(wp + 4);
          const f32x2 w[4] = {f32x2{w0[0], w0[1]}, f32x2{w0[2], w0[3]}, f32x2{w1[0], w1[1]}, f32x2{w1[2], w1[3]}};
#pragma unroll
          for (int k = 0; k < 4; ++k) {
            const float d = dd[k + 2 - kx];
            const f32x2 d2 = {d, d};
#pragma unroll
            for (int j = 0; j < 4; ++j) acc[k][j] += d2 * w[j];
          }
        }
      }
    }
    u32x4 o8[4];
#pragma unroll
    for (int k = 0; k < 4; ++k) {
      bf16x8 v;
#pragma unroll
      for (int j = 0; j < 4; ++j) {
        v[2 * j] = (bf16)(scale * acc[k][j][0]);
        v[2 * j + 1] = (bf16)(scale * acc[k][j][1]);
      }
      o8[k] = __builtin_bit_cast(u32x4, v);
    }
#pragma unroll
    for (int k = 0; k < 4; ++k) {
      if (x0 + k < W) {
        const long e = (p + k) * C + c8 * 8;
        if (ga) *reinterpret_cast<u32x4*>(ga + e) = o8[k];
        if constexpr (FUSED) *reinterpret_cast<u32x4*>(gr + e) = mod_silu_drop_bwd8(o8[k], ub[k], e >> 3, mv, m, part);
      }
    }
  }
  if constexpr (FUSED) {
#pragma unroll
    for (int j = 0; j < 8; ++j) red[ps * C + c8 * 8 + j] = part[j];
    __syncthreads();
    for (int c = threadIdx.x; c < C; c += blockDim.x) {
      float s = 0.f;
      for (int q = 0; q < PS; ++q) s += red[q * C + c];
      atomicAdd(gm + (long)b * gm_stride + c, s);
    }
  }
}

template <int CO>
static int launch_dgrad(const float* dF, const float* Wc, float scale, void* ga, const void* U, const float* lin,
                        long lin_stride, const float* gain, void* gr, float* gm, long gm_stride, float pdrop,
                        unsigned long long seed, unsigned sub, unsigned step, int u_marked, int B, int H, int W, int C,
                        const void* dyn, hipStream_t st) {
  const int CL = C / 8, block = (256 / CL) * CL, PS = block / CL;
  const int NSX = (W + 3) / 4, TP = NSX * 4 + 4;
  int R = 128 / W;
  R = R < 1 ? 1 : (R > H ? H : R);
  auto lds = [&](int r) { return dgrad_lds(CO, C, W, r, U != nullptr); };
  while (R > 1 && lds(R) > LOWRANK_LDS_MAX) --R;
  EDM_REQUIRE(lds(R) <= LOWRANK_LDS_MAX, "lowrank_dgrad3x3: Co=%d, C=%d, W=%d need %zu bytes of LDS (60 KB at most)", CO, C, W,
              lds(R));
  const dim3 grid((H + R - 1) / R, B);
  if (U)
    hipLaunchKernelGGL((k_lowrank_dgrad3x3<CO, true>), grid, dim3(block), lds(R), st, dF, Wc, scale, (bf16*)ga,
                       (const bf16*)U, lin, lin_stride, gain, (bf16*)gr, gm, gm_stride, pdrop, (uint32_t)seed,
                       (uint32_t)(seed >> 32), sub, step, u_marked, (const StepParams*)dyn, H, W, C, R, TP);
  else
    hipLaunchKernelGGL((k_lowrank_dgrad3x3<CO, false>), grid, dim3(block), lds(R), st, dF, Wc, scale, (bf16*)ga,
                       (const bf16*)nullptr, (const float*)nullptr, 0L, (const float*)nullptr, (bf16*)nullptr,
                       (float*)nullptr, 0L, 0.f, 0u, 0u, 0u, 0u, 0, (const StepParams*)nullptr, H, W, C, R, TP);
  EDM_CHECK_LAUNCH("lowrank_dgrad3x3");
  return EDM_OK;
}

#define EDM_CO_SWITCH(Co, CALL)      \
  switch (Co) {                      \
    case 1: return CALL(1);          \
    case 2: return CALL(2);          \
    case 3: return CALL(3);          \
    case 4: return CALL(4);          \
    case 5: return CALL(5);          \
    case 6: return CALL(6);          \
    case 7: return CALL(7);          \
    default: return CALL(8);         \
  }

extern "C" int edm_lowrank_dgrad3x3(const float* dF, const float* Wc, float scale, void* ga, const void* r1,
                                    const float* lin, long lin_stride, const float* gain, void* gr, float* gm,
                                    long gm_stride, float pdrop, unsigned long long seed, unsigned sub, unsigned step,
                                    int u_marked, int B, int H, int W, int C, int Co, const void* dyn, hipStream_t st) {
  EDM_REQUIRE(dF && Wc && (ga || r1), "lowrank_dgrad3x3: null pointer");
  EDM_REQUIRE(B > 0 && B <= 65535 && H > 0 && W > 0 && C > 0 && C % 8 == 0 && C <= 2048 && Co >= 1 && Co <= 8,
              "lowrank_dgrad3x3: bad args (C %% 8 == 0, Co <= 8 required)");
  EDM_REQUIRE(((uintptr_t)Wc & 15) == 0, "lowrank_dgrad3x3: Wc must be 16-byte aligned");
  if (r1)
    EDM_REQUIRE(lin && gain && gr && gm && lin_stride >= C && gm_stride >= C && pdrop >= 0.f && pdrop < 1.f,
                "lowrank_dgrad3x3: bad modulation-backward args");
#define CALL(CO_) launch_dgrad<CO_>(dF, Wc, scale, ga, r1, lin, lin_stride, gain, gr, gm, gm_stride, pdrop, seed, sub, step, \
                                    u_marked, B, H, W, C, dyn, st)
  EDM_CO_SWITCH(Co, CALL)
#undef CALL
}

template <int CO, int TAPS, int VEC>
__global__ __launch_bounds__(512) void k_lowrank_wgrad(const float* __restrict__ dF, const bf16* __restrict__ X,
                                                       const float* __restrict__ aux, float* __restrict__ ws, int H,
                                                       int W, int C, int R, int upb, int nunits) {
  constexpr int HALO = TAPS == 9 ? 1 : 0, K = TAPS == 9 ? 3 : 1, NB = 8;
  extern __shared__ __attribute__((aligned(16))) float sm[];
  __shared__ float asums[512];
  const int N = CO * TAPS * C, TPW = W + 2 * HALO, TR = R + 2 * HALO;
  float* accl = sm;
  float* tl = sm + N;
  typedef __attribute__((ext_vector_type(VEC / 2))) unsigned int uraw;
  const int CLV = C / VEC;
  const int PS = blockDim.x / CLV;
  const int cv = threadIdx.x % CLV, ps = threadIdx.x / CLV;
  f32x2 acc[CO * TAPS][VEC / 2];
#pragma unroll
  for (int e = 0; e < CO * TAPS; ++e)
#pragma unroll
    for (int h = 0; h < VEC / 2; ++h) acc[e][h] = f32x2{0.f, 0.f};
  float asum = 0.f;
  for (int u = blockIdx.x; u < nunits; u += gridDim.x) {
    const int b = u / upb, y0 = (u - b * upb) * R;
    const int rows = min(R, H - y0);
    __syncthreads();
    for (int i = threadIdx.x; i < CO * TR * TPW; i += blockDim.x) {
      const int o = i / (TR * TPW), rem = i - o * TR * TPW;
      const int ry = rem / TPW, cx = rem - ry * TPW;
      const int y = y0 + ry - HALO, x = cx - HALO;
      float v = 0.f;
      if (y >= 0 && y < H && x >= 0 && x < W)
        v = dF[(((long)b * CO + o) * H + y) * W + x];
      tl[i] = v;
    }
    if (aux) {
      for (int o = 0; o < CO; ++o) {
        const float* ap = aux + (((long)b * CO + o) * H + y0) * W;
        for (int i = threadIdx.x; i < rows * W; i += blockDim.x) asum += ap[i];
      }
    }
    __syncthreads();
    const int np = rows * W;
    const bf16* xp = X + (((long)b * H + y0) * W) * C + cv * VEC;
    int ry = ps / W, x = ps - (ps / W) * W;
    uraw nx[NB];
    auto fetch = [&](int q0) {
#pragma unroll
      for (int i = 0; i < NB; ++i) {
        const int q = q0 + i * PS;
        nx[i] = uraw{};
        if (q < np) nx[i] = *reinterpret_cast<const uraw*>(xp + (long)q * C);
      }
    };
    fetch(ps);
    for (int q0 = ps; q0 < np; q0 += NB * PS) {
      uraw cur[NB];
#pragma unroll
      for (int i = 0; i < NB; ++i) cur[i] = nx[i];
      if (q0 + NB * PS < np) fetch(q0 + NB * PS);
#pragma unroll
      for (int i = 0; i < NB; ++i) {
        if (q0 + i * PS < np) {
          typedef __attribute__((ext_vector_type(VEC))) __bf16 bfv;
          const bfv xv = __builtin_bit_cast(bfv, cur[i]);
          f32x2 xf[VEC / 2];
#pragma unroll
          for (int h = 0; h < VEC / 2; ++h) xf[h] = f32x2{(float)xv[2 * h], (float)xv[2 * h + 1]};
#pragma unroll
          for (int o = 0; o < CO; ++o)
#pragma unroll
            for (int ky = 0; ky < K; ++ky)
#pragma unroll
              for (int kx = 0; kx < K; ++kx) {
                const float d = tl[(o * TR + ry + 2 * HALO - ky) * TPW + x + 2 * HALO - kx];
                const f32x2 d2 = {d, d};
#pragma unroll
                for (int h = 0; h < VEC / 2; ++h) acc[o * TAPS + ky * K + kx][h] += d2 * xf[h];
              }
        }
        x += PS;
        while (x >= W) {
          x -= W;
          ++ry;
        }
      }
    }
  }
  for (int r = 0; r < PS; ++r) {
    __syncthreads();
    if (ps == r) {
#pragma unroll
      for (int e = 0; e < CO * TAPS; ++e) {
#pragma unroll
        for (int h = 0; h < VEC / 2; ++h) {
          f32x2* ap = reinterpret_cast<f32x2*>(accl + e * C + cv * VEC + 2 * h);
          f32x2 v = acc[e][h];
          if (r) v += *ap;
          *ap = v;
        }
      }
    }
  }
  asums[threadIdx.x] = asum;
  __syncthreads();
  float* row = ws + (long)blockIdx.x * (N + 4);
  for (int i = threadIdx.x; i < N; i += blockDim.x) row[i] = accl[i];
  if (threadIdx.x == 0) {
    float s = 0.f;
    for (int i = 0; i < (int)blockDim.x; ++i) s += asums[i];
    row[N] = s;
  }
}

__global__ __launch_bounds__(1024) void k_lowrank_reduce(const float* __restrict__ ws, int nwg, int N, float* __restrict__ G,
                                                         float* __restrict__ aux_out) {
  __shared__ float part[16][64];
  const int l = threadIdx.x & 63, seg = threadIdx.x >> 6;
  const int e = blockIdx.x * 64 + l;
  const int per = (nwg + 15) / 16;
  const int r0 = seg * per;
  float v[16];
#pragma unroll
  for (int k = 0; k < 16; ++k) {
    const int r = r0 + k;
    v[k] = (e <= N && k < per && r < nwg) ? ws[(long)r * (N + 4) + e] : 0.f;
  }
  float s = 0.f;
#pragma unroll
  for (int k = 0; k < 16; ++k) s += v[k];
  part[seg][l] = s;
  __syncthreads();
  if (seg == 0 && e <= N) {
    float t = 0.f;
#pragma unroll
    for (int k = 0; k < 16; ++k) t += part[k][l];
    if (e < N) G[e] = t;
    else if (aux_out) *aux_out += t;
  }
}

template <int CO>
static int launch_wgrad(const float* dF, const void* X, int taps, const float* aux, float* G, float* aux_out, float* ws,
                        long ws_floats, int B, int H, int W, int C, int nwg, hipStream_t st) {
  constexpr int VEC = CO <= 4 ? 4 : 2;
  const int CLV = C / VEC;
  int PS = 512 / CLV;
  PS = PS > 16 ? 16 : PS;
  const int block = PS * CLV, halo = taps == 9 ? 1 : 0;
  const int N = CO * taps * C;
  int R = 512 / W;
  R = R < 1 ? 1 : (R > H ? H : R);
  auto lds = [&](int r) { return wgrad_lds(CO, taps, C, W, r); };
  while (R > 1 && lds(R) > LOWRANK_LDS_MAX) --R;
  EDM_REQUIRE(lds(R) <= LOWRANK_LDS_MAX, "lowrank_wgrad: Co=%d, taps=%d, C=%d, W=%d need %zu bytes of LDS (60 KB at most)", CO,
              taps, C, W, lds(R));
  const int upb = (H + R - 1) / R;
  EDM_REQUIRE((long)B * upb < (1L << 31), "lowrank_wgrad: too many units");
  const int nunits = B * upb;
  const int grid = nunits < nwg ? nunits : nwg;
  EDM_REQUIRE(ws_floats >= (long)grid * (N + 4), "lowrank_wgrad: workspace of %ld floats, %ld needed", ws_floats,
              (long)grid * (N + 4));
  if (taps == 9)
    hipLaunchKernelGGL((k_lowrank_wgrad<CO, 9, VEC>), dim3(grid), dim3(block), lds(R), st, dF, (const bf16*)X, aux, ws, H, W, C,
                       R, upb, nunits);
  else
    hipLaunchKernelGGL((k_lowrank_wgrad<CO, 1, VEC>), dim3(grid), dim3(block), lds(R), st, dF, (const bf16*)X, aux, ws, H, W, C,
                       R, upb, nunits);
  EDM_CHECK_LAUNCH("lowrank_wgrad");
  hipLaunchKernelGGL(k_lowrank_reduce, dim3((N + 1 + 63) / 64), dim3(1024), 0, st, ws, grid, N, G, aux_out);
  EDM_CHECK_LAUNCH("lowrank_reduce");
  return EDM_OK;
}

constexpr int LOWRANK_WGRAD_NWG = 256;
extern "C" long edm_lowrank_wgrad_workspace(int C, int Co, int taps) {
  return (long)LOWRANK_WGRAD_NWG * ((long)Co * taps * C + 4);
}

extern "C" int edm_lowrank_wgrad(const float* dF, const void* X, int taps, const float* aux, float* G, float* aux_out,
                                 float* ws, long ws_floats, int B, int H, int W, int C, int Co, hipStream_t st) {
  EDM_REQUIRE(dF && X && G && ws && (!aux || aux_out), "lowrank_wgrad: null pointer");
  EDM_REQUIRE(B > 0 && H > 0 && W > 0 && C > 0 && C % 8 == 0 && C <= 1024 && Co >= 1 && Co <= 8 && (taps == 1 || taps == 9),
              "lowrank_wgrad: bad args (C %% 8 == 0, Co <= 8, taps 1 or 9 required)");
#define CALL(CO_) launch_wgrad<CO_>(dF, X, taps, aux, G, aux_out, ws, ws_floats, B, H, W, C, LOWRANK_WGRAD_NWG, st)
  EDM_CO_SWITCH(Co, CALL)
#undef CALL
}

__global__ void k_lowrank_expand_wc(const float* __restrict__ wout, const bf16* __restrict__ wd, float* __restrict__ Wc,
                                    int Co, int O, int I, int taps) {
  const int lane = threadIdx.x & 63;
  const int row = blockIdx.x * (blockDim.x >> 6) + (threadIdx.x >> 6);
  if (row >= taps * I) return;
  const int tt = row / I, ci = row - tt * I;
  float acc[8] = {0, 0, 0, 0, 0, 0, 0, 0};
  for (int c = lane * 8; c < O; c += 64 * 8) {
    float v[8];
    load8(wd + (long)row * O + c, v);
#pragma unroll
    for (int o = 0; o < 8; ++o)
      if (o < Co) {
#pragma unroll
        for (int j = 0; j < 8; ++j) acc[o] += wout[(long)o * O + c + j] * v[j];
      }
  }
#pragma unroll
  for (int o = 0; o < 8; ++o)
    if (o < Co) {
      const float s = wave_sum(acc[o]);
      if (lane == 0) Wc[((long)o * taps + (taps - 1 - tt)) * I + ci] = s;
    }
}
extern "C" int edm_lowrank_expand_wc(const float* wout_hat, const void* wd, float* Wc, int Co, int O, int I, int taps,
                                     hipStream_t st) {
  EDM_REQUIRE(wout_hat && wd && Wc, "lowrank_expand_wc: null pointer");
  EDM_REQUIRE(Co >= 1 && Co <= 8 && O > 0 && O % 8 == 0 && I > 0 && taps >= 1, "lowrank_expand_wc: bad args");
  hipLaunchKernelGGL(k_lowrank_expand_wc, dim3((taps * I + 3) / 4), dim3(256), 0, st, wout_hat, (const bf16*)wd, Wc, Co, O,
                     I, taps);
  EDM_CHECK_LAUNCH("lowrank_expand_wc");
  return EDM_OK;
}

__global__ void k_lowrank_expand_slab(const float* __restrict__ wout, const float* __restrict__ G, float* __restrict__ slab,
                                      float scale, int Co, int O, int I, int Ipad, int taps, long n) {
  for (long e = (long)blockIdx.x * blockDim.x + threadIdx.x; e < n; e += (long)gridDim.x * blockDim.x) {
    const int i = (int)(e % Ipad);
    const long tc = e / Ipad;
    const int c = (int)(tc % O), t = (int)(tc / O);
    float s = 0.f;
    if (i < I)
      for (int o = 0; o < Co; ++o) s += wout[(long)o * O + c] * G[((long)o * taps + t) * I + i];
    slab[e] = scale * s;
  }
}
extern "C" int edm_lowrank_expand_slab(const float* wout_hat, const float* G, float* slab, float scale, int Co, int O, int I,
                                       int Ipad, int taps, hipStream_t st) {
  EDM_REQUIRE(wout_hat && G && slab, "lowrank_expand_slab: null pointer");
  EDM_REQUIRE(Co >= 1 && Co <= 8 && O > 0 && I > 0 && Ipad >= I && taps >= 1, "lowrank_expand_slab: bad args");
  const long n = (long)taps * O * Ipad;
  const long blocks = (n + 255) / 256;
  hipLaunchKernelGGL(k_lowrank_expand_slab, dim3((unsigned)(blocks < 4096 ? blocks : 4096)), dim3(256), 0, st, wout_hat, G,
                     slab, scale, Co, O, I, Ipad, taps, n);
  EDM_CHECK_LAUNCH("lowrank_expand_slab");
  return EDM_OK;
}

constexpr int TAIL_LPP = 8;
static size_t tail_fwd_lds(int Co, int C, int Cc, int W, int R) {
  return ((size_t)Co * 9 * C + (size_t)Co * Cc + (size_t)R * W * 10 * Co) * sizeof(float);
}
extern "C" int edm_lowrank_tail_supported(int C, int Cc, int Co, int W) {
  if (C <= 0 || C % 8 || C > 1024 || Cc <= 0 || Cc % 8 || Cc > 2048 || Co < 1 || Co > 8 || W <= 0) return 0;
  return tail_fwd_lds(Co, C, Cc, W, 1) <= LOWRANK_LDS_MAX;
}

template <int CO, int NK, int PX>
__device__ __forceinline__ void tail_dots(const bf16* const (&xp)[PX], int Cx, const float* __restrict__ w, int wso, int lig,
                                          float (&s)[PX][NK * CO]) {
  f32x2 acc[PX][NK * CO];
#pragma unroll
  for (int k = 0; k < PX; ++k)
#pragma unroll
    for (int v = 0; v < NK * CO; ++v) acc[k][v] = f32x2{0.f, 0.f};
  const int CL = Cx >> 3;
  for (int c8 = lig; c8 < CL; c8 += TAIL_LPP) {
    f32x2 xf[PX][4];
#pragma unroll
    for (int k = 0; k < PX; ++k) {
      u32x4 raw = u32x4{0u, 0u, 0u, 0u};
      if (xp[k]) raw = *reinterpret_cast<const u32x4*>(xp[k] + c8 * 8);
      const bf16x8 xv = __builtin_bit_cast(bf16x8, raw);
#pragma unroll
      for (int h = 0; h < 4; ++h) xf[k][h] = f32x2{(float)xv[2 * h], (float)xv[2 * h + 1]};
    }
#pragma unroll
    for (int o = 0; o < CO; ++o)
#pragma unroll
      for (int kk = 0; kk < NK; ++kk) {
        const float* wp = w + (long)(o * wso + kk) * Cx + c8 * 8;
        const f32x4 w0 = *reinterpret_cast<const f32x4*>(wp), w1 = *reinterpret_cast<const f32x4*>(wp + 4);
        const f32x2 wv[4] = {f32x2{w0[0], w0[1]}, f32x2{w0[2], w0[3]}, f32x2{w1[0], w1[1]}, f32x2{w1[2], w1[3]}};
#pragma unroll
        for (int k = 0; k < PX; ++k)
#pragma unroll
          for (int h = 0; h < 4; ++h) acc[k][kk * CO + o] += xf[k][h] * wv[h];
      }
  }
#pragma unroll
  for (int k = 0; k < PX; ++k)
#pragma unroll
    for (int v = 0; v < NK * CO; ++v) s[k][v] = group_sum<TAIL_LPP>(acc[k][v][0] + acc[k][v][1]);
}

template <int CO, int PX>
__global__ __launch_bounds__(512) void k_lowrank_tail_fwd(const bf16* __restrict__ a2, const bf16* __restrict__ cat,
                                                          const float* __restrict__ Wc, const float* __restrict__ Wp,
                                                          float sb, float sa, const float* __restrict__ gain_out,
                                                          const float* __restrict__ noisy, const float* __restrict__ sigma,
                                                          int sstride, float sd, float* __restrict__ D,
                                                          float* __restrict__ Fraw, int H, int W, int C, int Cc, int R) {
  extern __shared__ __attribute__((aligned(16))) float sm[];
  float* wl = sm;
  float* wpl = wl + CO * 9 * C;
  float* pt = wpl + CO * Cc;
  const int RW = R * W;
  float* qt = pt + 3 * RW * 3 * CO;
  const int b = blockIdx.y, y0 = blockIdx.x * R;
  const int rows = min(R, H - y0);
  for (int i = threadIdx.x; i < CO * 9 * C / 4; i += blockDim.x)
    reinterpret_cast<f32x4*>(wl)[i] = reinterpret_cast<const f32x4*>(Wc)[i];
  for (int i = threadIdx.x; i < CO * Cc / 4; i += blockDim.x)
    reinterpret_cast<f32x4*>(wpl)[i] = reinterpret_cast<const f32x4*>(Wp)[i];
  __syncthreads();
  const int lig = threadIdx.x % TAIL_LPP, grp = threadIdx.x / TAIL_LPP, NG = blockDim.x / TAIL_LPP;
#pragma unroll 1
  for (int ky = 0; ky < 3; ++ky) {
    const int r_lo = max(y0 + ky - 1, 0), r_hi = min(y0 + rows - 1 + ky - 1, H - 1);
    const int np = (r_hi - r_lo + 1) * W;
    const int slot0 = (r_lo - (y0 + ky - 1)) * W;
    const bf16* base = a2 + (((long)b * H + r_lo) * W) * C;
    float* po = pt + (long)ky * RW * 3 * CO;
    for (int n0 = grp * PX; n0 < np; n0 += NG * PX) {
      const bf16* xp[PX];
#pragma unroll
      for (int k = 0; k < PX; ++k) xp[k] = n0 + k < np ? base + (long)(n0 + k) * C : nullptr;
      float s[PX][3 * CO];
      tail_dots<CO, 3, PX>(xp, C, wl + ky * 3 * C, 9, lig, s);
#pragma unroll
      for (int k = 0; k < PX; ++k)
        if (n0 + k < np) {
#pragma unroll
          for (int v = 0; v < 3 * CO; ++v)
            if ((v % TAIL_LPP) == lig) po[(long)(slot0 + n0 + k) * 3 * CO + v] = s[k][v];
        }
    }
  }
  {
    const int np = rows * W;
    const bf16* base = cat + (((long)b * H + y0) * W) * Cc;
    for (int n0 = grp * PX; n0 < np; n0 += NG * PX) {
      const bf16* xp[PX];
#pragma unroll
      for (int k = 0; k < PX; ++k) xp[k] = n0 + k < np ? base + (long)(n0 + k) * Cc : nullptr;
      float s[PX][CO];
      tail_dots<CO, 1, PX>(xp, Cc, wpl, 1, lig, s);
#pragma unroll
      for (int k = 0; k < PX; ++k)
        if (n0 + k < np) {
#pragma unroll
          for (int v = 0; v < CO; ++v)
            if ((v % TAIL_LPP) == lig) qt[(long)(n0 + k) * CO + v] = s[k][v];
        }
    }
  }
  __syncthreads();
  const float go = *gain_out;
  const float sg = sigma[b * sstride];
  const float den = sg * sg + sd * sd;
  const float cskip = sd * sd / den, cout = sg * sd * rsqrtf(den);
  for (int i = threadIdx.x; i < CO * rows * W; i += blockDim.x) {
    const int o = i / (rows * W), n = i - o * rows * W;
    const int ry = n / W, x = n - ry * W;
    float s = 0.f;
#pragma unroll
    for (int ky = 0; ky < 3; ++ky) {
      const int iy = y0 + ry + ky - 1;
      if (iy < 0 || iy >= H) continue;
#pragma unroll
      for (int kx = 0; kx < 3; ++kx) {
        const int ix = x + kx - 1;
        if (ix < 0 || ix >= W) continue;
        s += pt[((long)ky * RW + ry * W + ix) * 3 * CO + kx * CO + o];
      }
    }
    const float f = sb * s + sa * qt[(long)n * CO + o];
    const long idx = (((long)b * CO + o) * H + y0 + ry) * W + x;
    if (Fraw) Fraw[idx] = f;
    D[idx] = f * go * cout + noisy[idx] * cskip;
  }
}

template <int CO>
static int launch_tail_fwd(const void* a2, const void* cat, const float* Wc, const float* Wp, float sb, float sa,
                           const float* gain_out, const float* noisy, const float* sigma, int sstride, float sd, float* D,
                           float* Fraw, int B, int H, int W, int C, int Cc, hipStream_t st) {
  constexpr int PX = CO <= 4 ? 2 : 1;
  int R = 128 / W;
  R = R < 1 ? 1 : (R > H ? H : R);
  auto lds = [&](int r) { return tail_fwd_lds(CO, C, Cc, W, r); };
  while (R > 1 && lds(R) > LOWRANK_LDS_MAX) --R;
  EDM_REQUIRE(lds(R) <= LOWRANK_LDS_MAX, "lowrank_tail_fwd: Co=%d, C=%d, Cc=%d, W=%d need %zu bytes of LDS (60 KB at most)", CO,
              C, Cc, W, lds(R));
  const long want = ((long)(R + 1) * W + PX - 1) / PX * TAIL_LPP;
  int block = want >= 512 ? 512 : (int)((want + 63) / 64 * 64);
  const dim3 grid((H + R - 1) / R, B);
  hipLaunchKernelGGL((k_lowrank_tail_fwd<CO, PX>), grid, dim3(block), lds(R), st, (const bf16*)a2, (const bf16*)cat, Wc, Wp, sb,
                     sa, gain_out, noisy, sigma, sstride, sd, D, Fraw, H, W, C, Cc, R);
  EDM_CHECK_LAUNCH("lowrank_tail_fwd");
  return EDM_OK;
}

extern "C" int edm_lowrank_tail_fwd(const void* a2, const void* cat, const float* Wc, const float* Wp, float sb, float sa,
                                    const float* gain_out, const float* noisy, const float* sigma, int sigma_stride,
                                    float sigma_data, float* D, float* Fraw, int B, int H, int W, int C, int Cc, int Co,
                                    hipStream_t st) {
  EDM_REQUIRE(a2 && cat && Wc && Wp && gain_out && noisy && sigma && D, "lowrank_tail_fwd: null pointer");
  EDM_REQUIRE(B > 0 && B <= 65535 && H > 0 && W > 0 && (sigma_stride == 0 || sigma_stride == 1), "lowrank_tail_fwd: bad args");
  EDM_REQUIRE(edm_lowrank_tail_supported(C, Cc, Co, W), "lowrank_tail_fwd: unsupported shape C=%d Cc=%d Co=%d W=%d", C, Cc, Co, W);
  EDM_REQUIRE((((uintptr_t)Wc | (uintptr_t)Wp | (uintptr_t)a2 | (uintptr_t)cat) & 15) == 0,
              "lowrank_tail_fwd: operands must be 16-byte aligned");
#define CALL(CO_) launch_tail_fwd<CO_>(a2, cat, Wc, Wp, sb, sa, gain_out, noisy, sigma, sigma_stride, sigma_data, D, Fraw, B, \
                                       H, W, C, Cc, st)
  EDM_CO_SWITCH(Co, CALL)
#undef CALL
}

__global__ __launch_bounds__(256) void k_lowrank_tail_dwout(const float* __restrict__ G, const bf16* __restrict__ wf2,
                                                            const float* __restrict__ G1, const bf16* __restrict__ wf1,
                                                            float sb, float sa, float* __restrict__ gwh, int Co, int C,
                                                            int Cc) {
  const int lane = threadIdx.x & 63;
  const int c = blockIdx.x * (blockDim.x >> 6) + (threadIdx.x >> 6);
  if (c >= C) return;
  float a9[8] = {0, 0, 0, 0, 0, 0, 0, 0}, a1[8] = {0, 0, 0, 0, 0, 0, 0, 0};
  for (int t = 0; t < 9; ++t)
    for (int ci = lane * 8; ci < C; ci += 64 * 8) {
      float v[8];
      load8(wf2 + ((long)t * C + c) * C + ci, v);
#pragma unroll
      for (int o = 0; o < 8; ++o)
        if (o < Co) {
          const float* gp = G + ((long)o * 9 + t) * C + ci;
#pragma unroll
          for (int j = 0; j < 8; ++j) a9[o] += v[j] * gp[j];
        }
    }
  if (wf1)
    for (int cj = lane * 8; cj < Cc; cj += 64 * 8) {
      float v[8];
      load8(wf1 + (long)c * Cc + cj, v);
#pragma unroll
      for (int o = 0; o < 8; ++o)
        if (o < Co) {
          const float* gp = G1 + (long)o * Cc + cj;
#pragma unroll
          for (int j = 0; j < 8; ++j) a1[o] += v[j] * gp[j];
        }
    }
#pragma unroll
  for (int o = 0; o < 8; ++o)
    if (o < Co) {
      const float s9 = wave_sum(a9[o]);
      const float s1 = wf1 ? wave_sum(a1[o]) : G1[(long)o * Cc + c];
      if (lane == 0) gwh[(long)o * C + c] = sb * s9 + sa * s1;
    }
}
extern "C" int edm_lowrank_tail_dwout_supported(int C, int Cc, int Co, int has1) {
  return C > 0 && C % 8 == 0 && Cc > 0 && Cc % 8 == 0 && Co >= 1 && Co <= 8 && (has1 || Cc == C);
}
extern "C" int edm_lowrank_tail_dwout(const float* G, const void* wf2, const float* G1, const void* wf1, float sb, float sa,
                                      float* gwh, int Co, int C, int Cc, hipStream_t st) {
  EDM_REQUIRE(G && wf2 && G1 && gwh, "lowrank_tail_dwout: null pointer");
  EDM_REQUIRE(edm_lowrank_tail_dwout_supported(C, Cc, Co, wf1 != nullptr), "lowrank_tail_dwout: bad args (C=%d Cc=%d Co=%d)", C, Cc,
              Co);
  EDM_REQUIRE((((uintptr_t)wf2 | (uintptr_t)wf1) & 15) == 0, "lowrank_tail_dwout: packs must be 16-byte aligned");
  hipLaunchKernelGGL(k_lowrank_tail_dwout, dim3((C + 3) / 4), dim3(256), 0, st, G, (const bf16*)wf2, G1, (const bf16*)wf1, sb,
                     sa, gwh, Co, C, Cc);
  EDM_CHECK_LAUNCH("lowrank_tail_dwout");
  return EDM_OK;
}

__global__ void k_lowrank_gcat_add(const float* __restrict__ dF, const float* __restrict__ Wp, float sa,
                                   const bf16* __restrict__ t, bf16* __restrict__ gu, bf16* __restrict__ gcs, int HW, int Cc,
                                   int Ci, int Co, long n8) {
  const unsigned CL = (unsigned)Cc >> 3, uHW = (unsigned)HW, CiL = (unsigned)Ci >> 3;
  for (unsigned i = blockIdx.x * blockDim.x + threadIdx.x; i < (unsigned)n8; i += gridDim.x * blockDim.x) {
    const unsigned p = i / CL, c8 = i - p * CL;
    const unsigned b = p / uHW, hw = p - b * uHW;
    float v[8] = {0, 0, 0, 0, 0, 0, 0, 0}, tv[8];
    load8(t + (long)i * 8, tv);
    for (int o = 0; o < Co; ++o) {
      const float df = dF[((long)b * Co + o) * HW + hw];
      const float* wp = Wp + (long)o * Cc + c8 * 8;
#pragma unroll
      for (int j = 0; j < 8; ++j) v[j] += df * wp[j];
    }
#pragma unroll
    for (int j = 0; j < 8; ++j) v[j] = tv[j] + sa * v[j];
    if (c8 < CiL) store8(gu + ((long)p * Ci + c8 * 8), v);
    else store8(gcs + ((long)p * (Cc - Ci) + (c8 - CiL) * 8), v);
  }
}
extern "C" int edm_lowrank_gcat_supported(int Cc, int Ci, int Co) {
  return Cc > 0 && Cc % 8 == 0 && Ci > 0 && Ci % 8 == 0 && Ci <= Cc && Co >= 1 && Co <= 8;
}
extern "C" int edm_lowrank_gcat_add(const float* dF, const float* Wp, float sa, const void* t, void* gu, void* gcs, int B,
                                    int HW, int Cc, int Ci, int Co, hipStream_t st) {
  EDM_REQUIRE(dF && Wp && t && gu, "lowrank_gcat_add: null pointer");
  EDM_REQUIRE(B > 0 && HW > 0 && edm_lowrank_gcat_supported(Cc, Ci, Co) && (gcs || Ci == Cc),
              "lowrank_gcat_add: bad args (Cc=%d Ci=%d Co=%d)", Cc, Ci, Co);
  const long n8 = (long)B * HW * (Cc / 8);
  EDM_REQUIRE(n8 < (1L << 31), "lowrank_gcat_add: too many elements");
  const long blocks = (n8 + 255) / 256;
  hipLaunchKernelGGL(k_lowrank_gcat_add, dim3((unsigned)(blocks < 8192 ? blocks : 8192)), dim3(256), 0, st, dF, Wp, sa,
                     (const bf16*)t, (bf16*)gu, (bf16*)gcs, HW, Cc, Ci, Co, n8);
  EDM_CHECK_LAUNCH("lowrank_gcat_add");
  return EDM_OK;
}
```

Before: 10290 img/s.

## Add occupancy-tuned skip-gate kernels, gate sorting, wgrad modes, and tail prefetch

Templates the skip-gate forward and backward kernels with a TWO variant. That variant uses smaller reduce unroll, launch bounds targeting two blocks per CU, and register-cached gate values with batched loads in the elementwise tail. Gate items are sorted by spatial size so large-HW blocks are scheduled first. The low-rank wgrad kernel gains parallel accumulation modes with precomputed offsets. The tail forward gets software prefetch of the next channel chunk, and tail dwout preloads its weights using one wave per block. Each change sits behind an environment switch that is on by default, which adds register-pressure and LDS-layout risk.

```diff
diff --git a/tinyedm_amd/csrc/elementwise.hip b/tinyedm_amd/csrc/elementwise.hip
--- a/tinyedm_amd/csrc/elementwise.hip
+++ b/tinyedm_amd/csrc/elementwise.hip
@@ -1,4 +1,5 @@
 #include "common.h"
+#include <algorithm>
 #include <stdarg.h>
 #include <stdio.h>
 
@@ -713,7 +714,7 @@
   return EDM_OK;
 }
 
-template <bool MUL>
+template <bool MUL, int UN = 8>
 __device__ __forceinline__ void sample_reduce(const bf16* __restrict__ x, long xs, const bf16* __restrict__ y, long ys,
                                               int HW, int C, float* red, float* out_lds, float scale) {
   const int lpr = C >> 3;
@@ -721,7 +722,6 @@
   const int cl = threadIdx.x % lpr, rg = threadIdx.x / lpr;
   float acc[8] = {0, 0, 0, 0, 0, 0, 0, 0};
   if (rg < rpp) {
-    constexpr int UN = 8;
     for (int p0 = rg; p0 < HW; p0 += rpp * UN) {
       u32x4 v[UN], u[UN];
 #pragma unroll
@@ -756,7 +756,7 @@
   __syncthreads();
 }
 
-template <bool KEEP = false>
+template <bool KEEP = false, int UN = 8>
 __device__ __forceinline__ void skip_gate_fwd_body(const bf16* __restrict__ skip, const float* __restrict__ W1,
                                                    const float* __restrict__ W2, float* __restrict__ mean,
                                                    float* __restrict__ gate, float* __restrict__ z1save, int HW,
@@ -766,7 +766,7 @@
   float* red = sm;
   float* m = sm + rpp * C;
   float* h = m + C + 1;
-  sample_reduce<false>(skip + (long)b * HW * C, C, nullptr, 0, HW, C, red, m, 1.0f / (float)HW);
+  sample_reduce<false, UN>(skip + (long)b * HW * C, C, nullptr, 0, HW, C, red, m, 1.0f / (float)HW);
   for (int c = threadIdx.x; c < C; c += blockDim.x) mean[(long)b * C + c] = m[c];
   if (threadIdx.x == 0) m[C] = 1.0f;
   __syncthreads();
@@ -810,13 +810,15 @@
   SgfItem it[MAXSGF];
   int n, C, pad[2];
 };
-__global__ __launch_bounds__(1024) void k_skip_gate_fwd_multi(const SgfGroup* __restrict__ g) {
+constexpr int SG_U = 4;
+template <bool TWO>
+__global__ __launch_bounds__(1024, TWO ? 8 : 4) void k_skip_gate_fwd_multi(const SgfGroup* __restrict__ g) {
   int k = 0;
   const int n = g->n;
   while (k + 1 < n && (int)blockIdx.x >= g->it[k + 1].blk0) ++k;
   const SgfItem it = g->it[k];
   const int C = g->C, b = (int)blockIdx.x - it.blk0;
-  skip_gate_fwd_body<true>(it.skip, it.W1, it.W2, it.mean, it.gate, it.z1, it.HW, C, it.R, b);
+  skip_gate_fwd_body<true, TWO ? 4 : 8>(it.skip, it.W1, it.W2, it.mean, it.gate, it.z1, it.HW, C, it.R, b);
   if (it.cat == nullptr) return;
   __syncthreads();
   extern __shared__ __attribute__((aligned(16))) float sm[];
@@ -825,22 +827,53 @@
   const bf16* __restrict__ sk = it.skip + (long)b * it.HW * C;
   bf16* __restrict__ cat = it.cat + (long)b * it.HW * ld + it.Ci;
   bf16* __restrict__ sil = it.sil ? it.sil + (long)b * it.HW * ld + it.Ci : nullptr;
-  const int n8 = it.HW * CLs;
-  for (int i = threadIdx.x; i < n8; i += blockDim.x) {
-    const int cs = (i % CLs) * 8;
-    const int pix = i / CLs;
-    float v[8];
-    load8(sk + (long)pix * C + cs, v);
-#pragma unroll
-    for (int j = 0; j < 8; ++j) v[j] = (float)(bf16)(v[j] * sm[cs + j]);
-    store8(cat + (long)pix * ld + cs, v);
-    if (sil) {
-#pragma unroll
-      for (int j = 0; j < 8; ++j) v[j] = mp_silu_b(v[j]);
-      store8(sil + (long)pix * ld + cs, v);
-    }
-  }
-}
+  if constexpr (!TWO) {
+    const int n8 = it.HW * CLs;
+    for (int i = threadIdx.x; i < n8; i += blockDim.x) {
+      const int cs = (i % CLs) * 8;
+      const int pix = i / CLs;
+      float v[8];
+      load8(sk + (long)pix * C + cs, v);
+#pragma unroll
+      for (int j = 0; j < 8; ++j) v[j] = (float)(bf16)(v[j] * sm[cs + j]);
+      store8(cat + (long)pix * ld + cs, v);
+      if (sil) {
+#pragma unroll
+        for (int j = 0; j < 8; ++j) v[j] = mp_silu_b(v[j]);
+        store8(sil + (long)pix * ld + cs, v);
+      }
+    }
+  } else {
+    const int rpp = blockDim.x / CLs, cs = (threadIdx.x % CLs) * 8, HW = it.HW;
+    float gt[8];
+#pragma unroll
+    for (int j = 0; j < 8; ++j) gt[j] = sm[cs + j];
+    for (int p0 = threadIdx.x / CLs; p0 < HW; p0 += rpp * SG_U) {
+      u32x4 raw[SG_U];
+#pragma unroll
+      for (int u = 0; u < SG_U; ++u) {
+        const int pix = p0 + u * rpp;
+        if (pix < HW) raw[u] = *reinterpret_cast<const u32x4*>(sk + (long)pix * C + cs);
+      }
+#pragma unroll
+      for (int u = 0; u < SG_U; ++u) {
+        const int pix = p0 + u * rpp;
+        if (pix >= HW) break;
+        const bf16x8 a = __builtin_bit_cast(bf16x8, raw[u]);
+        float v[8];
+#pragma unroll
+        for (int j = 0; j < 8; ++j) v[j] = (float)(bf16)((float)a[j] * gt[j]);
+        store8(cat + (long)pix * ld + cs, v);
+        if (sil) {
+#pragma unroll
+          for (int j = 0; j < 8; ++j) v[j] = mp_silu_b(v[j]);
+          store8(sil + (long)pix * ld + cs, v);
+        }
+      }
+    }
+  }
+}
+template <int UN = 8>
 __device__ __forceinline__ void skip_gate_bwd_body(const bf16* __restrict__ gcat, long gs, const bf16* __restrict__ skip,
                                                    const float* __restrict__ W1, const float* __restrict__ W2,
                                                    const float* __restrict__ gate, const float* __restrict__ z1save,
@@ -852,7 +885,7 @@
   float* gz2 = sm + rpp * C;
   float* gz1 = gz2 + C;
   float* wsb = ws + (long)b * (C + 2 * R);
-  sample_reduce<true>(gcat + (long)b * HW * gs, gs, skip + (long)b * HW * C, C, HW, C, red, gz2, 1.0f);
+  sample_reduce<true, UN>(gcat + (long)b * HW * gs, gs, skip + (long)b * HW * C, C, HW, C, red, gz2, 1.0f);
   for (int c = threadIdx.x; c < C; c += blockDim.x) {
     const float g = gate[(long)b * C + c];
     gz2[c] *= g * (1.0f - g);
@@ -897,13 +930,14 @@
   SgbItem it[MAXSGF];
   int n, C, pad[2];
 };
-__global__ __launch_bounds__(1024) void k_skip_gate_bwd_multi(const SgbGroup* __restrict__ g) {
+template <bool TWO>
+__global__ __launch_bounds__(1024, TWO ? 8 : 4) void k_skip_gate_bwd_multi(const SgbGroup* __restrict__ g) {
   int k = 0;
   const int n = g->n;
   while (k + 1 < n && (int)blockIdx.x >= g->it[k + 1].blk0) ++k;
   const SgbItem it = g->it[k];
   const int C = g->C, b = (int)blockIdx.x - it.blk0;
-  skip_gate_bwd_body(it.gcat, it.gs, it.skip, it.W1, it.W2, it.gate, it.z1, it.gmean, it.ws, it.HW, C, it.R, b);
+  skip_gate_bwd_body<TWO ? 2 : 8>(it.gcat, it.gs, it.skip, it.W1, it.W2, it.gate, it.z1, it.gmean, it.ws, it.HW, C, it.R, b);
   if (it.gskip == nullptr) return;
   __syncthreads();
   const int CLs = C >> 3;
@@ -912,17 +946,45 @@
   bf16* __restrict__ out = it.gskip + (long)b * it.HW * C;
   const float* gp0 = it.gate + (long)b * C;
   const float* mp0 = it.gmean + (long)b * C;
-  const int n8 = it.HW * CLs;
-  for (int i = threadIdx.x; i < n8; i += blockDim.x) {
-    const int cs = (i % CLs) * 8;
-    const int pix = i / CLs;
-    float v[8];
-    load8(gc + (long)pix * it.gs + cs, v);
-    const float* gp = gp0 + cs;
-    const float* mp = mp0 + cs;
-#pragma unroll
-    for (int j = 0; j < 8; ++j) v[j] = v[j] * gp[j] + mp[j] * inv_hw;
-    store8(out + (long)pix * C + cs, v);
+  if constexpr (!TWO) {
+    const int n8 = it.HW * CLs;
+    for (int i = threadIdx.x; i < n8; i += blockDim.x) {
+      const int cs = (i % CLs) * 8;
+      const int pix = i / CLs;
+      float v[8];
+      load8(gc + (long)pix * it.gs + cs, v);
+      const float* gp = gp0 + cs;
+      const float* mp = mp0 + cs;
+#pragma unroll
+      for (int j = 0; j < 8; ++j) v[j] = v[j] * gp[j] + mp[j] * inv_hw;
+      store8(out + (long)pix * C + cs, v);
+    }
+  } else {
+    const int rpp = blockDim.x / CLs, cs = (threadIdx.x % CLs) * 8, HW = it.HW;
+    float gp[8], mp[8];
+#pragma unroll
+    for (int j = 0; j < 8; ++j) {
+      gp[j] = gp0[cs + j];
+      mp[j] = mp0[cs + j];
+    }
+    for (int p0 = threadIdx.x / CLs; p0 < HW; p0 += rpp * SG_U) {
+      u32x4 raw[SG_U];
+#pragma unroll
+      for (int u = 0; u < SG_U; ++u) {
+        const int pix = p0 + u * rpp;
+        if (pix < HW) raw[u] = *reinterpret_cast<const u32x4*>(gc + (long)pix * it.gs + cs);
+      }
+#pragma unroll
+      for (int u = 0; u < SG_U; ++u) {
+        const int pix = p0 + u * rpp;
+        if (pix >= HW) break;
+        const bf16x8 a = __builtin_bit_cast(bf16x8, raw[u]);
+        float v[8];
+#pragma unroll
+        for (int j = 0; j < 8; ++j) v[j] = (float)a[j] * gp[j] + mp[j] * inv_hw;
+        store8(out + (long)pix * C + cs, v);
+      }
+    }
   }
 }
 __device__ __forceinline__ void skip_gate_wgrad_body(const float* __restrict__ ws, const float* __restrict__ mean,
@@ -1002,6 +1064,16 @@
   const int lpr = C / 8;
   int t = 1024 / lpr * lpr;
   return t < 64 ? 0 : t;
+}
+static inline bool sg_switch(const char* name) {
+  const char* e = getenv(name);
+  return !(e && e[0] == '0');
+}
+template <class Item>
+static inline void sg_order(const Item* items, int n, int* order) {
+  for (int k = 0; k < n; ++k) order[k] = k;
+  if (!sg_switch("EDM_GATE_SORT")) return;
+  std::stable_sort(order, order + n, [&](int a, int b) { return items[a].HW > items[b].HW; });
 }
 extern "C" int edm_skip_gate_fwd(const void* skip, const float* W1h, const float* W2h, float* mean, float* gate,
                                  float* z1save, int B, int HW, int C, int R, hipStream_t st) {
@@ -1041,14 +1113,17 @@
   EDM_REQUIRE(threads > 0, "skip_gate_fwd_multi: C too large");
   long blk = 0;
   int rmax = 0;
-  for (int k = 0; k < n; ++k) {
+  int order[MAXSGF];
+  sg_order(items, n, order);
+  for (int s = 0; s < n; ++s) {
+    const int k = order[s];
     const edm_skip_gate_fwd_item_& a = items[k];
     EDM_REQUIRE(a.skip && a.W1h && a.W2h && a.mean && a.gate && a.z1save, "skip_gate_fwd_multi: null pointer (gate %d)", k);
     EDM_REQUIRE(a.C == C, "skip_gate_fwd_multi: the gates of one launch share a channel count (%d vs %d)", a.C, C);
     EDM_REQUIRE(a.B > 0 && a.HW > 0 && a.R > 0 && a.R <= 1024, "skip_gate_fwd_multi: bad item %d", k);
     EDM_REQUIRE(a.cat ? (a.Ci > 0 && a.Ci % 8 == 0) : (a.silu_out == nullptr),
                 "skip_gate_fwd_multi: cat needs Ci %% 8 == 0 (gate %d); silu_out needs cat", k);
-    g.it[k] = SgfItem{(const bf16*)a.skip, a.W1h, a.W2h, a.mean, a.gate, a.z1save, (bf16*)a.cat, (bf16*)a.silu_out, a.Ci, 0,
+    g.it[s] = SgfItem{(const bf16*)a.skip, a.W1h, a.W2h, a.mean, a.gate, a.z1save, (bf16*)a.cat, (bf16*)a.silu_out, a.Ci, 0,
                       a.B, a.HW, a.R, (int)blk};
     blk += a.B;
     EDM_REQUIRE(blk < (1L << 30), "skip_gate_fwd_multi: grid too large");
@@ -1058,7 +1133,10 @@
     g.it[k] = SgfItem{nullptr, nullptr, nullptr, nullptr, nullptr, nullptr, nullptr, nullptr, 0, 0, 0, 0, 0, (int)blk};
   const size_t lds = ((size_t)(threads / (C / 8)) * C + C + 1 + rmax) * sizeof(float);
   EDM_UPLOAD_TABLE(table_dev, table_host, &g, sizeof(SgfGroup), st, "skip_gate_fwd_multi", defer_upload);
-  hipLaunchKernelGGL(k_skip_gate_fwd_multi, dim3((unsigned)blk), dim3(threads), lds, st, (const SgfGroup*)table_dev);
+  if (sg_switch("EDM_GATE_TWO"))
+    hipLaunchKernelGGL(k_skip_gate_fwd_multi<true>, dim3((unsigned)blk), dim3(threads), lds, st, (const SgfGroup*)table_dev);
+  else
+    hipLaunchKernelGGL(k_skip_gate_fwd_multi<false>, dim3((unsigned)blk), dim3(threads), lds, st, (const SgfGroup*)table_dev);
   EDM_CHECK_LAUNCH("skip_gate_fwd_multi");
   return EDM_OK;
 }
@@ -1110,14 +1188,17 @@
   EDM_REQUIRE(threads > 0, "skip_gate_bwd_multi: C too large");
   long blk = 0;
   int rmax = 0;
-  for (int k = 0; k < n; ++k) {
+  int order[MAXSGF];
+  sg_order(items, n, order);
+  for (int s = 0; s < n; ++s) {
+    const int k = order[s];
     const edm_skip_gate_bwd_item_& a = items[k];
     EDM_REQUIRE(a.gcat && a.skip && a.W1h && a.W2h && a.gate && a.z1save && a.gmean && a.ws,
                 "skip_gate_bwd_multi: null pointer (gate %d)", k);
     EDM_REQUIRE(a.C == C, "skip_gate_bwd_multi: the gates of one launch share a channel count (%d vs %d)", a.C, C);
     EDM_REQUIRE(a.B > 0 && a.HW > 0 && a.R > 0 && a.R <= 1024 && a.c_off >= 0 && a.c_off % 8 == 0 &&
                     a.gcat_stride >= a.c_off + C && a.gcat_stride % 8 == 0, "skip_gate_bwd_multi: bad item %d", k);
-    g.it[k] = SgbItem{(const bf16*)a.gcat + a.c_off, a.gcat_stride, (const bf16*)a.skip, a.W1h, a.W2h, a.gate, a.z1save,
+    g.it[s] = SgbItem{(const bf16*)a.gcat + a.c_off, a.gcat_stride, (const bf16*)a.skip, a.W1h, a.W2h, a.gate, a.z1save,
                       a.gmean, a.ws, (bf16*)a.gskip, a.B, a.HW, a.R, (int)blk};
     blk += a.B;
     EDM_REQUIRE(blk < (1L << 30), "skip_gate_bwd_multi: grid too large");
@@ -1127,7 +1208,10 @@
     g.it[k] = SgbItem{nullptr, 0, nullptr, nullptr, nullptr, nullptr, nullptr, nullptr, nullptr, nullptr, 0, 0, 0, (int)blk};
   const size_t lds = ((size_t)(threads / (C / 8)) * C + C + rmax) * sizeof(float);
   EDM_UPLOAD_TABLE(table_dev, table_host, &g, sizeof(SgbGroup), st, "skip_gate_bwd_multi", defer_upload);
-  hipLaunchKernelGGL(k_skip_gate_bwd_multi, dim3((unsigned)blk), dim3(threads), lds, st, (const SgbGroup*)table_dev);
+  if (sg_switch("EDM_GATE_TWO"))
+    hipLaunchKernelGGL(k_skip_gate_bwd_multi<true>, dim3((unsigned)blk), dim3(threads), lds, st, (const SgbGroup*)table_dev);
+  else
+    hipLaunchKernelGGL(k_skip_gate_bwd_multi<false>, dim3((unsigned)blk), dim3(threads), lds, st, (const SgbGroup*)table_dev);
   EDM_CHECK_LAUNCH("skip_gate_bwd_multi");
   return EDM_OK;
 }
diff --git a/tinyedm_amd/csrc/tail_lowrank.hip b/tinyedm_amd/csrc/tail_lowrank.hip
--- a/tinyedm_amd/csrc/tail_lowrank.hip
+++ b/tinyedm_amd/csrc/tail_lowrank.hip
@@ -10,6 +10,11 @@
 static size_t wgrad_lds(int Co, int taps, int C, int W, int R) {
   const int halo = taps == 9 ? 1 : 0;
   return ((size_t)Co * taps * C + (size_t)Co * (R + 2 * halo) * (W + 2 * halo)) * sizeof(float);
+}
+static constexpr int wgrad_ec(int Co, int taps) { return (Co * taps) % 3 == 0 ? 3 : 1; }
+static size_t wgrad_lds_par(int Co, int taps, int C, int W, int R, int PS) {
+  const int halo = taps == 9 ? 1 : 0;
+  return ((size_t)wgrad_ec(Co, taps) * PS * C + (size_t)Co * (R + 2 * halo) * (W + 2 * halo)) * sizeof(float);
 }
 extern "C" int edm_lowrank_supported(int C, int Co, int W, int taps) {
   if (C <= 0 || C % 8 || C > 1024 || Co < 1 || Co > 8 || W <= 0 || (taps != 1 && taps != 9)) return 0;
@@ -214,7 +219,7 @@
 #undef CALL
 }
 
-template <int CO, int TAPS, int VEC>
+template <int CO, int TAPS, int VEC, int MODE>
 __global__ __launch_bounds__(512) void k_lowrank_wgrad(const float* __restrict__ dF, const bf16* __restrict__ X,
                                                        const float* __restrict__ aux, float* __restrict__ ws, int H,
                                                        int W, int C, int R, int upb, int nunits) {
@@ -223,11 +228,22 @@
   __shared__ float asums[512];
   const int N = CO * TAPS * C, TPW = W + 2 * HALO, TR = R + 2 * HALO;
   float* accl = sm;
-  float* tl = sm + N;
+  float* tl = sm + (MODE > 0 ? wgrad_ec(CO, TAPS) * (int)(blockDim.x / (C / VEC)) * C : N);
   typedef __attribute__((ext_vector_type(VEC / 2))) unsigned int uraw;
   const int CLV = C / VEC;
   const int PS = blockDim.x / CLV;
-  const int cv = threadIdx.x % CLV, ps = threadIdx.x / CLV;
+  const int cv = threadIdx.x % CLV;
+  const int ps = MODE == 2 ? __builtin_amdgcn_readfirstlane(threadIdx.x / CLV) : threadIdx.x / CLV;
+  constexpr int NT = CO * TAPS, NDV = (NT + 63) / 64;
+  int doff[NDV];
+  if constexpr (MODE == 2) {
+#pragma unroll
+    for (int j = 0; j < NDV; ++j) {
+      const int e0 = j * 64 + (int)(threadIdx.x & 63), e = e0 < NT ? e0 : 0;
+      const int o = e / TAPS, t = e - o * TAPS, ky = t / K, kx = t - ky * K;
+      doff[j] = (o * TR + 2 * HALO - ky) * TPW + 2 * HALO - kx;
+    }
+  }
   f32x2 acc[CO * TAPS][VEC / 2];
 #pragma unroll
   for (int e = 0; e < CO * TAPS; ++e)
@@ -237,6 +253,17 @@
   for (int u = blockIdx.x; u < nunits; u += gridDim.x) {
     const int b = u / upb, y0 = (u - b * upb) * R;
     const int rows = min(R, H - y0);
+    const int np = rows * W;
+    const bf16* xp = X + (((long)b * H + y0) * W) * C + cv * VEC;
+    uraw nx[NB];
+    auto fetch = [&](int q0) {
+#pragma unroll
+      for (int i = 0; i < NB; ++i) {
+        const int q = q0 + i * PS;
+        nx[i] = uraw{};
+        if (q < np) nx[i] = *reinterpret_cast<const uraw*>(xp + (long)q * C);
+      }
+    };
     __syncthreads();
     for (int i = threadIdx.x; i < CO * TR * TPW; i += blockDim.x) {
       const int o = i / (TR * TPW), rem = i - o * TR * TPW;
@@ -254,18 +281,7 @@
       }
     }
     __syncthreads();
-    const int np = rows * W;
-    const bf16* xp = X + (((long)b * H + y0) * W) * C + cv * VEC;
     int ry = ps / W, x = ps - (ps / W) * W;
-    uraw nx[NB];
-    auto fetch = [&](int q0) {
-#pragma unroll
-      for (int i = 0; i < NB; ++i) {
-        const int q = q0 + i * PS;
-        nx[i] = uraw{};
-        if (q < np) nx[i] = *reinterpret_cast<const uraw*>(xp + (long)q * C);
-      }
-    };
     fetch(ps);
     for (int q0 = ps; q0 < np; q0 += NB * PS) {
       uraw cur[NB];
@@ -280,6 +296,18 @@
           f32x2 xf[VEC / 2];
 #pragma unroll
           for (int h = 0; h < VEC / 2; ++h) xf[h] = f32x2{(float)xv[2 * h], (float)xv[2 * h + 1]};
+          if constexpr (MODE == 2) {
+            float dv[NDV];
+#pragma unroll
+            for (int j = 0; j < NDV; ++j) dv[j] = tl[ry * TPW + x + doff[j]];
+#pragma unroll
+            for (int e = 0; e < NT; ++e) {
+              const float d = __builtin_bit_cast(float, __builtin_amdgcn_readlane(__builtin_bit_cast(int, dv[e / 64]), e % 64));
+              const f32x2 d2 = {d, d};
+#pragma unroll
+              for (int h = 0; h < VEC / 2; ++h) acc[e][h] += d2 * xf[h];
+            }
+          } else
 #pragma unroll
           for (int o = 0; o < CO; ++o)
 #pragma unroll
@@ -300,6 +328,35 @@
       }
     }
   }
+  float* row = ws + (long)blockIdx.x * (N + 4);
+  if constexpr (MODE > 0) {
+    constexpr int EC = wgrad_ec(CO, TAPS);
+    float* sc = sm;
+#pragma unroll
+    for (int e0 = 0; e0 < NT; e0 += EC) {
+      __syncthreads();
+#pragma unroll
+      for (int j = 0; j < EC; ++j)
+#pragma unroll
+        for (int h = 0; h < VEC / 2; ++h)
+          *reinterpret_cast<f32x2*>(sc + (j * PS + ps) * C + cv * VEC + 2 * h) = acc[e0 + j][h];
+      __syncthreads();
+      for (int i = threadIdx.x; i < EC * C; i += blockDim.x) {
+        const int j = i / C, c = i - j * C;
+        float v = sc[(j * PS) * C + c];
+        for (int r = 1; r < PS; ++r) v = sc[(j * PS + r) * C + c] + v;
+        row[(e0 + j) * C + c] = v;
+      }
+    }
+    asums[threadIdx.x] = asum;
+    __syncthreads();
+    if (threadIdx.x == 0) {
+      float s = 0.f;
+      for (int i = 0; i < (int)blockDim.x; ++i) s += asums[i];
+      row[N] = s;
+    }
+    return;
+  }
   for (int r = 0; r < PS; ++r) {
     __syncthreads();
     if (ps == r) {
@@ -317,7 +374,6 @@
   }
   asums[threadIdx.x] = asum;
   __syncthreads();
-  float* row = ws + (long)blockIdx.x * (N + 4);
   for (int i = threadIdx.x; i < N; i += blockDim.x) row[i] = accl[i];
   if (threadIdx.x == 0) {
     float s = 0.f;
@@ -362,24 +418,35 @@
   PS = PS > 16 ? 16 : PS;
   const int block = PS * CLV, halo = taps == 9 ? 1 : 0;
   const int N = CO * taps * C;
+  const char* env = getenv("EDM_TAIL_WGRAD");
+  int mode = env && env[0] == '0' ? 0 : (CLV % 64 == 0 ? 2 : 1);
   int R = 512 / W;
   R = R < 1 ? 1 : (R > H ? H : R);
-  auto lds = [&](int r) { return wgrad_lds(CO, taps, C, W, r); };
-  while (R > 1 && lds(R) > LOWRANK_LDS_MAX) --R;
-  EDM_REQUIRE(lds(R) <= LOWRANK_LDS_MAX, "lowrank_wgrad: Co=%d, taps=%d, C=%d, W=%d need %zu bytes of LDS (60 KB at most)", CO,
-              taps, C, W, lds(R));
+  auto lds0 = [&](int r) { return wgrad_lds(CO, taps, C, W, r); };
+  while (R > 1 && lds0(R) > LOWRANK_LDS_MAX) --R;
+  if (mode && wgrad_lds_par(CO, taps, C, W, R, PS) > LOWRANK_LDS_MAX) mode = 0;
+  auto lds = [&](int r) { return mode ? wgrad_lds_par(CO, taps, C, W, r, PS) : lds0(r); };
+  EDM_REQUIRE(lds0(R) <= LOWRANK_LDS_MAX, "lowrank_wgrad: Co=%d, taps=%d, C=%d, W=%d need %zu bytes of LDS (60 KB at most)", CO,
+              taps, C, W, lds0(R));
   const int upb = (H + R - 1) / R;
   EDM_REQUIRE((long)B * upb < (1L << 31), "lowrank_wgrad: too many units");
   const int nunits = B * upb;
   const int grid = nunits < nwg ? nunits : nwg;
   EDM_REQUIRE(ws_floats >= (long)grid * (N + 4), "lowrank_wgrad: workspace of %ld floats, %ld needed", ws_floats,
               (long)grid * (N + 4));
-  if (taps == 9)
-    hipLaunchKernelGGL((k_lowrank_wgrad<CO, 9, VEC>), dim3(grid), dim3(block), lds(R), st, dF, (const bf16*)X, aux, ws, H, W, C,
-                       R, upb, nunits);
-  else
-    hipLaunchKernelGGL((k_lowrank_wgrad<CO, 1, VEC>), dim3(grid), dim3(block), lds(R), st, dF, (const bf16*)X, aux, ws, H, W, C,
-                       R, upb, nunits);
+#define LAUNCH(TAPS_, MODE_)                                                                                              \
+  hipLaunchKernelGGL((k_lowrank_wgrad<CO, TAPS_, VEC, MODE_>), dim3(grid), dim3(block), lds(R), st, dF, (const bf16*)X, aux, \
+                     ws, H, W, C, R, upb, nunits)
+  if (taps == 9) {
+    if (mode == 2) LAUNCH(9, 2);
+    else if (mode == 1) LAUNCH(9, 1);
+    else LAUNCH(9, 0);
+  } else {
+    if (mode == 2) LAUNCH(1, 2);
+    else if (mode == 1) LAUNCH(1, 1);
+    else LAUNCH(1, 0);
+  }
+#undef LAUNCH
   EDM_CHECK_LAUNCH("lowrank_wgrad");
   hipLaunchKernelGGL(k_lowrank_reduce, dim3((N + 1 + 63) / 64), dim3(1024), 0, st, ws, grid, N, G, aux_out);
   EDM_CHECK_LAUNCH("lowrank_reduce");
@@ -468,7 +535,7 @@
   return tail_fwd_lds(Co, C, Cc, W, 1) <= LOWRANK_LDS_MAX;
 }
 
-template <int CO, int NK, int PX>
+template <int CO, int NK, int PX, bool PF>
 __device__ __forceinline__ void tail_dots(const bf16* const (&xp)[PX], int Cx, const float* __restrict__ w, int wso, int lig,
                                           float (&s)[PX][NK * CO]) {
   f32x2 acc[PX][NK * CO];
@@ -477,12 +544,29 @@
 #pragma unroll
     for (int v = 0; v < NK * CO; ++v) acc[k][v] = f32x2{0.f, 0.f};
   const int CL = Cx >> 3;
+  u32x4 nxt[PX];
+  if constexpr (PF) {
+#pragma unroll
+    for (int k = 0; k < PX; ++k) {
+      nxt[k] = u32x4{0u, 0u, 0u, 0u};
+      if (xp[k] && lig < CL) nxt[k] = *reinterpret_cast<const u32x4*>(xp[k] + lig * 8);
+    }
+  }
   for (int c8 = lig; c8 < CL; c8 += TAIL_LPP) {
     f32x2 xf[PX][4];
+    u32x4 cur[PX];
+    if constexpr (PF) {
+#pragma unroll
+      for (int k = 0; k < PX; ++k) {
+        cur[k] = nxt[k];
+        if (xp[k] && c8 + TAIL_LPP < CL) nxt[k] = *reinterpret_cast<const u32x4*>(xp[k] + (c8 + TAIL_LPP) * 8);
+      }
+    }
 #pragma unroll
     for (int k = 0; k < PX; ++k) {
       u32x4 raw = u32x4{0u, 0u, 0u, 0u};
-      if (xp[k]) raw = *reinterpret_cast<const u32x4*>(xp[k] + c8 * 8);
+      if constexpr (PF) raw = cur[k];
+      else if (xp[k]) raw = *reinterpret_cast<const u32x4*>(xp[k] + c8 * 8);
       const bf16x8 xv = __builtin_bit_cast(bf16x8, raw);
 #pragma unroll
       for (int h = 0; h < 4; ++h) xf[k][h] = f32x2{(float)xv[2 * h], (float)xv[2 * h + 1]};
@@ -506,7 +590,7 @@
     for (int v = 0; v < NK * CO; ++v) s[k][v] = group_sum<TAIL_LPP>(acc[k][v][0] + acc[k][v][1]);
 }
 
-template <int CO, int PX>
+template <int CO, int PX, bool PF>
 __global__ __launch_bounds__(512) void k_lowrank_tail_fwd(const bf16* __restrict__ a2, const bf16* __restrict__ cat,
                                                           const float* __restrict__ Wc, const float* __restrict__ Wp,
                                                           float sb, float sa, const float* __restrict__ gain_out,
@@ -539,7 +623,7 @@
 #pragma unroll
       for (int k = 0; k < PX; ++k) xp[k] = n0 + k < np ? base + (long)(n0 + k) * C : nullptr;
       float s[PX][3 * CO];
-      tail_dots<CO, 3, PX>(xp, C, wl + ky * 3 * C, 9, lig, s);
+      tail_dots<CO, 3, PX, PF>(xp, C, wl + ky * 3 * C, 9, lig, s);
 #pragma unroll
       for (int k = 0; k < PX; ++k)
         if (n0 + k < np) {
@@ -557,7 +641,7 @@
 #pragma unroll
       for (int k = 0; k < PX; ++k) xp[k] = n0 + k < np ? base + (long)(n0 + k) * Cc : nullptr;
       float s[PX][CO];
-      tail_dots<CO, 1, PX>(xp, Cc, wpl, 1, lig, s);
+      tail_dots<CO, 1, PX, PF>(xp, Cc, wpl, 1, lig, s);
 #pragma unroll
       for (int k = 0; k < PX; ++k)
         if (n0 + k < np) {
@@ -608,8 +692,13 @@
   const long want = ((long)(R + 1) * W + PX - 1) / PX * TAIL_LPP;
   int block = want >= 512 ? 512 : (int)((want + 63) / 64 * 64);
   const dim3 grid((H + R - 1) / R, B);
-  hipLaunchKernelGGL((k_lowrank_tail_fwd<CO, PX>), grid, dim3(block), lds(R), st, (const bf16*)a2, (const bf16*)cat, Wc, Wp, sb,
-                     sa, gain_out, noisy, sigma, sstride, sd, D, Fraw, H, W, C, Cc, R);
+  const char* env = getenv("EDM_TAIL_FWD_PF");
+  if (env && env[0] == '0')
+    hipLaunchKernelGGL((k_lowrank_tail_fwd<CO, PX, false>), grid, dim3(block), lds(R), st, (const bf16*)a2, (const bf16*)cat, Wc,
+                       Wp, sb, sa, gain_out, noisy, sigma, sstride, sd, D, Fraw, H, W, C, Cc, R);
+  else
+    hipLaunchKernelGGL((k_lowrank_tail_fwd<CO, PX, true>), grid, dim3(block), lds(R), st, (const bf16*)a2, (const bf16*)cat, Wc,
+                       Wp, sb, sa, gain_out, noisy, sigma, sstride, sd, D, Fraw, H, W, C, Cc, R);
   EDM_CHECK_LAUNCH("lowrank_tail_fwd");
   return EDM_OK;
 }
@@ -629,6 +718,7 @@
 #undef CALL
 }
 
+template <bool PRE>
 __global__ __launch_bounds__(256) void k_lowrank_tail_dwout(const float* __restrict__ G, const bf16* __restrict__ wf2,
                                                             const float* __restrict__ G1, const bf16* __restrict__ wf1,
                                                             float sb, float sa, float* __restrict__ gwh, int Co, int C,
@@ -637,9 +727,24 @@
   const int c = blockIdx.x * (blockDim.x >> 6) + (threadIdx.x >> 6);
   if (c >= C) return;
   float a9[8] = {0, 0, 0, 0, 0, 0, 0, 0}, a1[8] = {0, 0, 0, 0, 0, 0, 0, 0};
+  u32x4 p9[9], p1 = u32x4{0u, 0u, 0u, 0u};
+  if constexpr (PRE) {
+#pragma unroll
+    for (int t = 0; t < 9; ++t) {
+      p9[t] = u32x4{0u, 0u, 0u, 0u};
+      if (lane * 8 < C) p9[t] = *reinterpret_cast<const u32x4*>(wf2 + ((long)t * C + c) * C + lane * 8);
+    }
+    if (wf1 && lane * 8 < Cc) p1 = *reinterpret_cast<const u32x4*>(wf1 + (long)c * Cc + lane * 8);
+  }
+#pragma unroll
   for (int t = 0; t < 9; ++t)
     for (int ci = lane * 8; ci < C; ci += 64 * 8) {
       float v[8];
+      if (PRE && ci == lane * 8) {
+        const bf16x8 pv = __builtin_bit_cast(bf16x8, p9[t]);
+#pragma unroll
+        for (int j = 0; j < 8; ++j) v[j] = (float)pv[j];
+      } else
       load8(wf2 + ((long)t * C + c) * C + ci, v);
 #pragma unroll
       for (int o = 0; o < 8; ++o)
@@ -652,6 +757,11 @@
   if (wf1)
     for (int cj = lane * 8; cj < Cc; cj += 64 * 8) {
       float v[8];
+      if (PRE && cj == lane * 8) {
+        const bf16x8 pv = __builtin_bit_cast(bf16x8, p1);
+#pragma unroll
+        for (int j = 0; j < 8; ++j) v[j] = (float)pv[j];
+      } else
       load8(wf1 + (long)c * Cc + cj, v);
 #pragma unroll
       for (int o = 0; o < 8; ++o)
@@ -678,8 +788,13 @@
   EDM_REQUIRE(edm_lowrank_tail_dwout_supported(C, Cc, Co, wf1 != nullptr), "lowrank_tail_dwout: bad args (C=%d Cc=%d Co=%d)", C, Cc,
               Co);
   EDM_REQUIRE((((uintptr_t)wf2 | (uintptr_t)wf1) & 15) == 0, "lowrank_tail_dwout: packs must be 16-byte aligned");
-  hipLaunchKernelGGL(k_lowrank_tail_dwout, dim3((C + 3) / 4), dim3(256), 0, st, G, (const bf16*)wf2, G1, (const bf16*)wf1, sb,
-                     sa, gwh, Co, C, Cc);
+  const char* env = getenv("EDM_TAIL_DWOUT");
+  if (env && env[0] == '0')
+    hipLaunchKernelGGL(k_lowrank_tail_dwout<false>, dim3((C + 3) / 4), dim3(256), 0, st, G, (const bf16*)wf2, G1,
+                       (const bf16*)wf1, sb, sa, gwh, Co, C, Cc);
+  else
+    hipLaunchKernelGGL(k_lowrank_tail_dwout<true>, dim3(C), dim3(64), 0, st, G, (const bf16*)wf2, G1, (const bf16*)wf1, sb, sa,
+                       gwh, Co, C, Cc);
   EDM_CHECK_LAUNCH("lowrank_tail_dwout");
   return EDM_OK;
 }
```

Result: no change. 10290 img/s (-0.0%).
